# jinggqu/NextGen-UIA

Hardware: AMD Instinct MI355X
Metric: images/sec fwd+bwd BiomedCLIP+Mona bs=256 (higher is better)
Workload: dtype bf16

## Files before the change

include/uia_hip.h:

```cpp
#ifndef UIA_HIP_H
#define UIA_HIP_H
#include <stddef.h>
#include <stdint.h>

#ifdef __cplusplus
extern "C" {
#endif

enum { UIA_F32 = 0, UIA_BF16 = 1 };
enum { UIA_ACT_NONE = 0, UIA_ACT_GELU = 1, UIA_ACT_QUICKGELU = 2, UIA_ACT_RELU = 3 };
enum { UIA_MASK_NONE = 0, UIA_MASK_CAUSAL = 1, UIA_MASK_KEYPAD = 2 };
enum { UIA_MONA_BASELINE = 0, UIA_MONA_NOISE_AWARE = 1, UIA_MONA_FREQ_ENHANCED = 2, UIA_MONA_HYBRID = 3 };

const char* uia_last_error(void);
int uia_version(void);

typedef struct uia_gemm_desc {
    const void* A; int64_t lda;
    const void* W; int64_t ldw;
    int32_t M, N, K;
    float alpha;
    const float* bias;
    int32_t act;
    int32_t dact;
    const void* aux_in; int64_t ldaux_in;
    void* aux_out; int64_t ldaux_out;
    const float* resid; int64_t ldr;
    int32_t resid_mod, resid_row_off;
    const void* residT; int64_t ldrT;
    int32_t out_group;
    void* outT; int64_t ldo;
    float* out32; int64_t ldo32;
    int32_t w_kblocked;
    const void* resid_ln_stats;
    const float* resid_ln_w;
    const float* resid_ln_b;
    int64_t* rowsum_out;
    const int64_t* lnfold_sums;
    const float* lnfold_colsum;
    int32_t lnfold_dim; float lnfold_eps;
    int32_t resid_ln_dim; float resid_ln_eps;
    int64_t a_kb_rows;
    int64_t outT_kb_rows;
    int32_t* ln_flag;
    float ln_flag_limit;
    int32_t drop_where;
    float drop_p;
    uint64_t drop_seed;
    void* a_drop_out;
    float* splitk_ws;
    const void* A2;
    int64_t lda2;
    int32_t K2;
    int32_t a2_group_cols;
    int64_t a2_group_stride;
    const int8_t* resid_lo8;
    int64_t ld_resid_lo;
    int64_t residT_kb_rows;
    int8_t* out_lo8;
    int64_t ld_out_lo;
    int64_t resid_lo_kb_rows;
    int64_t out_lo_kb_rows;
} uia_gemm_desc;
int uia_gemm(void* stream, int dtype, const uia_gemm_desc* d, int tile_cfg );

int uia_wgrad(void* stream, int dtype, int M, int I, int J, const void* A, int64_t lda, const void* B, int64_t ldb,
              float alpha, float* dW, float* dbias_A);
int uia_wgrad_ex(void* stream, int dtype, int M, int I, int J, const void* A, int64_t lda, const void* B, int64_t ldb,
                 float alpha, float* dW, int64_t ldw, int i_valid, int j_valid, float* dbias_A);
int uia_wgrad_drop(void* stream, int dtype, int M, int I, int J, const void* A, int64_t lda, const void* B, int64_t ldb,
                   float alpha, float* dW, int64_t ldw, int i_valid, int j_valid, float drop_p, uint64_t seed, int64_t drop_ld, int drop_col0);
typedef struct uia_wgrad_group_desc {
    int32_t n, M, I, J;
    const void* A[4];
    const void* B[4];
    float* dW[4];
    float* dbias_A[4];
    int64_t lda, ldb, ldw;
    int32_t i_valid, j_valid;
    float alpha, drop_p;
    uint64_t drop_seed[4];
    int64_t drop_ld;
    int32_t drop_col0, reserved;
} uia_wgrad_group_desc;
int uia_wgrad_group(void* stream, int dtype, const uia_wgrad_group_desc* d);

typedef struct uia_attn_desc {
    const void *q, *k, *v; int64_t ld_qkv;
    void* out; int64_t ldo;
    float* lse;
    const int32_t* keylen;
    int32_t B, H, L, dh;
    int32_t mask_kind;
// ... 286 lines not shown
```

nextgen-uia_amd/csrc/gemm.hip:

```cpp
#include "gemm_epilogue.h"

int uia_gemm_quad_launch(hipStream_t stream, const UiaGemmParams& p, bool specialise, int xflags);
int uia_gemm_quadv_launch(hipStream_t stream, const UiaGemmParams& p, bool specialise, int xflags, int depth);

namespace {

template <typename T, int BM, int BN, int WAVES_M, int WAVES_N>
__global__ __launch_bounds__(64 * WAVES_M * WAVES_N) void gemm_tn_kernel(const UiaGemmParams p) {
    extern __shared__ __attribute__((aligned(16))) char smem[];
    constexpr int NW = WAVES_M * WAVES_N;
    constexpr int WTM = BM / WAVES_M, WTN = BN / WAVES_N;
    constexpr int MT = WTM / 16, NT = WTN / 16;
    constexpr int A_BYTES = BM * 128, W_BYTES = BN * 128, BUF_BYTES = A_BYTES + W_BYTES;
    constexpr int A_PER_WAVE = (BM / 8) / NW, W_PER_WAVE = (BN / 8) / NW;
    static_assert((BM / 8) % NW == 0 && (BN / 8) % NW == 0, "staging must divide over the waves");
    static_assert(WTM % 16 == 0 && WTN % 16 == 0 && (NT % 2) == 0, "wave tile shape");
    constexpr int ESZ = (int)sizeof(T);

    const int tid = threadIdx.x, lane = tid & 63;
    const int wave = __builtin_amdgcn_readfirstlane(tid >> 6);
    const int wm = wave / WAVES_N, wn = wave % WAVES_N;

    const int tiles_n = (p.N + BN - 1) / BN;
    const int nwg = gridDim.x;
// ... 726 lines not shown
            if (t + PD < ntl) stage(t + PD);
            load_frags(buf);
            if (grp == 1 && t + 1 < ntl) retire(t + 1);
            UIA_SLOT_END();
            compute();
            if (grp == 0 && t + 1 < ntl) retire(t + 1);
            UIA_SLOT_END();
        }
        if (grp == 0) {
            UIA_SLOT_END();
        }
        const int cm0 = m0, cn0 = n0;
        const int next = tile + nslots;
        const bool more = next < t_hi;
        if (more) {
            point_at(next);
            for (int t = 0; t < PD && t < ntl; ++t) stage(t);
        }
        constexpr bool LNROW = EPI == EPI_GENERIC || (EPI & EPI_LNFOLD) != 0;
        gemm_epilogue_lds<T, MT, NT, WTM, WTN, EPI, true>(p, acc, smem + (NBUF - 1) * BUF_BYTES, wave, lane, cm0, cn0, wm, wn,
                                                          LNROW ? (float*)(smem + NBUF * BUF_BYTES + wave * (WTM * 8)) : nullptr);
        if (!more) break;
        tile = next;
    }
#undef UIA_SLOT_END
}

template <typename T, int EPI>
int launch_persist_epi(hipStream_t stream, const UiaGemmParams& p) {
    constexpr int LDS = 4 * 512 * 64 + ((EPI == EPI_GENERIC || (EPI & EPI_LNFOLD) != 0) ? 4 * 256 * 8 : 0);
    auto kern = gemm_tn_persist_kernel<T, EPI>;
    static UiaDevOnce attr_once;
    UIA_ENSURE_LDS_ATTR(attr_once, kern, LDS);
    const int tiles = ((p.M + 255) / 256) * ((p.N + 255) / 256);
    const int ncu = uia_num_cus();
    hipLaunchKernelGGL(kern, dim3(tiles < ncu ? tiles : ncu), dim3(512), LDS, stream, p);
    UIA_CHECK_LAUNCH();
    return 0;
}


template <typename T, int BM, int BN, int WAVES_M, int WAVES_N, int BKB, int NBUF, int LOOP = 0>
int launch_ring(hipStream_t stream, const UiaGemmParams& p, bool specialise, int xflags, int sk_info = 0) {
    if constexpr (BM == 128 && BN == 256 && NBUF == 4 && LOOP == 0) {
        if (sk_info != 0) return launch_ring_epi<T, BM, BN, WAVES_M, WAVES_N, BKB, NBUF, EPI_GENERIC, LOOP, true>(stream, p, xflags, sk_info);
    }
    if constexpr (BN == 256 && NBUF == 4 && LOOP == 0 && BKB == 64 && sizeof(T) == 2) {
        if (p.K2 > 0) {
            switch (epi_mask_of(p)) {
                case EPI_BIAS | EPI_OUTT: return launch_ring_epi<T, BM, BN, WAVES_M, WAVES_N, BKB, NBUF, (EPI_BIAS | EPI_OUTT), LOOP, false, true>(stream, p, xflags);
                case EPI_OUTT: return launch_ring_epi<T, BM, BN, WAVES_M, WAVES_N, BKB, NBUF, (EPI_OUTT), LOOP, false, true>(stream, p, xflags);
                case EPI_BIAS | EPI_RESID | EPI_OUT32: return launch_ring_epi<T, BM, BN, WAVES_M, WAVES_N, BKB, NBUF, (EPI_BIAS | EPI_RESID | EPI_OUT32), LOOP, false, true>(stream, p, xflags);
                default: return launch_ring_epi<T, BM, BN, WAVES_M, WAVES_N, BKB, NBUF, EPI_GENERIC, LOOP, false, true>(stream, p, xflags);
            }
        }
    }
    if (specialise) {
        switch (epi_mask_of(p)) {
#define UIA_EPI_CASE(MASK) case (MASK): return launch_ring_epi<T, BM, BN, WAVES_M, WAVES_N, BKB, NBUF, (MASK), LOOP>(stream, p, xflags)
            UIA_EPI_CASE(EPI_BIAS | EPI_RESID | EPI_OUT32);
            UIA_EPI_CASE(EPI_BIAS | EPI_RESIDT | EPI_OUT32);
            UIA_EPI_CASE(EPI_BIAS | EPI_RESID | EPI_RESID_LN | EPI_OUT32);
            UIA_EPI_CASE(EPI_OUTT);
            UIA_EPI_CASE(EPI_BIAS | EPI_OUTT);
            UIA_EPI_CASE(EPI_BIAS | EPI_GELU | EPI_OUTT);
            UIA_EPI_CASE(EPI_DGELU | EPI_OUTT);
            UIA_EPI_CASE(EPI_BIAS | EPI_GELU | EPI_AUX_OUT | EPI_OUTT);
            UIA_EPI_CASE(EPI_QUICK | EPI_BIAS | EPI_GELU | EPI_OUTT);
            UIA_EPI_CASE(EPI_QUICK | EPI_DGELU | EPI_OUTT);
            UIA_EPI_CASE(EPI_QUICK | EPI_BIAS | EPI_GELU | EPI_AUX_OUT | EPI_OUTT);
            UIA_EPI_CASE(EPI_BIAS | EPI_RESID | EPI_OUT32 | EPI_OUTT | EPI_ROWSUM);
            UIA_EPI_CASE(EPI_BIAS | EPI_RESID | EPI_RESID_LN | EPI_OUT32 | EPI_OUTT | EPI_ROWSUM);
            UIA_EPI_CASE(EPI_BIAS | EPI_RESID_LO | EPI_RESID_LN | EPI_OUTT | EPI_OUT_LO | EPI_ROWSUM);
            UIA_EPI_CASE(EPI_BIAS | EPI_RESID | EPI_OUTT | EPI_OUT_LO | EPI_ROWSUM);
            UIA_EPI_CASE(EPI_BIAS | EPI_RESID_LO | EPI_OUT32);
            UIA_EPI_CASE(EPI_BIAS | EPI_RESID | EPI_RESID_LN | EPI_OUTT | EPI_OUT_LO | EPI_ROWSUM);
            UIA_EPI_CASE(EPI_BIAS | EPI_RESID_LO | EPI_RESID_LN | EPI_OUT32);
            UIA_EPI_CASE(EPI_BIAS | EPI_RESID_LO | EPI_OUT32 | EPI_OUTT | EPI_ROWSUM);
            UIA_EPI_CASE(EPI_BIAS | EPI_OUTT | EPI_LNFOLD);
            UIA_EPI_CASE(EPI_BIAS | EPI_GELU | EPI_OUTT | EPI_LNFOLD);
            UIA_EPI_CASE(EPI_BIAS | EPI_GELU | EPI_AUX_OUT | EPI_OUTT | EPI_LNFOLD);
            UIA_EPI_CASE(EPI_QUICK | EPI_BIAS | EPI_GELU | EPI_OUTT | EPI_LNFOLD);
            UIA_EPI_CASE(EPI_QUICK | EPI_BIAS | EPI_GELU | EPI_AUX_OUT | EPI_OUTT | EPI_LNFOLD);
#undef UIA_EPI_CASE
            default: break;
        }
    }
    return launch_ring_epi<T, BM, BN, WAVES_M, WAVES_N, BKB, NBUF, EPI_GENERIC, LOOP>(stream, p, xflags);
}

template <typename T>
int launch_persist(hipStream_t stream, const UiaGemmParams& p) {
    switch (epi_mask_of(p)) {
#define UIA_EPI_CASE(MASK) case (MASK): return launch_persist_epi<T, (MASK)>(stream, p)
        UIA_EPI_CASE(EPI_BIAS | EPI_RESID | EPI_OUT32);
        UIA_EPI_CASE(EPI_BIAS | EPI_RESIDT | EPI_OUT32);
        UIA_EPI_CASE(EPI_OUTT);
        UIA_EPI_CASE(EPI_BIAS | EPI_OUTT);
        UIA_EPI_CASE(EPI_BIAS | EPI_GELU | EPI_OUTT);
        UIA_EPI_CASE(EPI_DGELU | EPI_OUTT);
        UIA_EPI_CASE(EPI_BIAS | EPI_GELU | EPI_AUX_OUT | EPI_OUTT);
        UIA_EPI_CASE(EPI_BIAS | EPI_OUTT | EPI_LNFOLD);
        UIA_EPI_CASE(EPI_BIAS | EPI_GELU | EPI_OUTT | EPI_LNFOLD);
        UIA_EPI_CASE(EPI_BIAS | EPI_GELU | EPI_AUX_OUT | EPI_OUTT | EPI_LNFOLD);
#undef UIA_EPI_CASE
        default: break;
    }
    return launch_persist_epi<T, EPI_GENERIC>(stream, p);
}

template <int CH, int NWV = 8>
__global__ __launch_bounds__(64 * NWV) void gemm_skinny64_kernel(const UiaGemmParams p) {
    extern __shared__ __attribute__((aligned(16))) char smem[];
    const int K = p.K, KS = K >> 5;
    const int ldw_b = 2 * K + 16;
    const int tid = threadIdx.x, lane = tid & 63, li = lane & 15, g = lane >> 4;
    const int wave = __builtin_amdgcn_readfirstlane(tid >> 6);
    {
        const int cpr = K >> 3;
        for (int c = tid; c < 64 * cpr; c += 64 * NWV) {
            const int r = c / cpr, cc = c - r * cpr;
            *(uint4*)(smem + r * ldw_b + cc * 16) = *(const uint4*)((const char*)p.W + ((size_t)r * p.ldw) * 2 + cc * 16);
        }
    }
    __syncthreads();
    float bias[4][4];
#pragma unroll
    for (int nt = 0; nt < 4; ++nt)
#pragma unroll
        for (int r = 0; r < 4; ++r) bias[nt][r] = p.bias ? p.bias[16 * nt + 4 * g + r] : 0.f;
    const char* wfrag = smem + li * ldw_b + g * 16;
    const bool drop_a = p.drop_where == 1;
    const uint32_t drop_th = dropout_thresh16(p.drop_p);
    const float drop_inv = 1.0f / (1.0f - p.drop_p);
    const int ntiles = (p.M + 15) >> 4;
    for (int tile = wave * gridDim.x + blockIdx.x; tile < ntiles; tile += gridDim.x * NWV) {
        const int m = 16 * tile + li;
        const int mc = m < p.M ? m : p.M - 1;
        const char* arow = (const char*)p.A + ((size_t)mc * p.lda) * 2 + g * 16;
        f32x4 acc[4] = {f32x4{0.f, 0.f, 0.f, 0.f}, f32x4{0.f, 0.f, 0.f, 0.f}, f32x4{0.f, 0.f, 0.f, 0.f}, f32x4{0.f, 0.f, 0.f, 0.f}};
        for (int ks0 = 0; ks0 < KS; ks0 += CH) {
            uint4 a[CH];
#pragma unroll
            for (int i = 0; i < CH; ++i) a[i] = ks0 + i < KS ? *(const uint4*)(arow + (ks0 + i) * 64) : uint4{0u, 0u, 0u, 0u};
            if (drop_a) {
#pragma unroll
                for (int i = 0; i < CH; ++i) {
                    if (ks0 + i < KS) {
                        const uint32_t keep = dropout_keep8(p.drop_seed, (uint32_t)(((size_t)mc * (size_t)K + (size_t)((ks0 + i) * 32 + g * 8)) >> 3), drop_th);
                        bf16x8 v = __builtin_bit_cast(bf16x8, a[i]);
#pragma unroll
                        for (int e = 0; e < 8; ++e) v[e] = (bf16_t)((keep >> e) & 1u ? (float)v[e] * drop_inv : 0.f);
                        a[i] = __builtin_bit_cast(uint4, v);
                        if (p.a_drop_out && m < p.M) *(uint4*)((char*)p.a_drop_out + ((size_t)m * p.lda) * 2 + g * 16 + (ks0 + i) * 64) = a[i];
                    }
                }
            }
#pragma unroll
            for (int i = 0; i < CH; ++i) {
                if (ks0 + i < KS) {
#pragma unroll
                    for (int nt = 0; nt < 4; ++nt) {
                        const uint4 wf = *(const uint4*)(wfrag + nt * 16 * ldw_b + (ks0 + i) * 64);
                        acc[nt] = __builtin_amdgcn_mfma_f32_16x16x32_bf16(__builtin_bit_cast(bf16x8, wf), __builtin_bit_cast(bf16x8, a[i]), acc[nt], 0, 0, 0);
                    }
                }
// ... 220 lines not shown
        return -1;
    }
    if (p.w_kblocked && !ring) {
        uia_set_error("uia_gemm: a K-blocked W needs a ring tile config (8, 9, 10, 13), not %d", cfg);
        return -1;
    }
    if (ring) {
        int gm = gm_req == 255 ? 0 : gm_req;
        if (gm_req == 0) gm = p.N >= 1536 ? 8 : 0;
        xflags = (xflags & ~255) | gm;
    }
    switch (cfg) {
        case 1: return launch_cfg<T, 256, 256, 2, 4>(stream, p);
        case 2: return launch_cfg<T, 256, 128, 4, 2>(stream, p);
        case 3: return launch_cfg<T, 128, 128, 2, 2>(stream, p);
        case 4: return launch_cfg<T, 256, 64, 4, 1>(stream, p);
        case 5: return launch_cfg<T, 128, 64, 2, 1>(stream, p);
        case 21: return launch_cfg<T, 32, 64, 2, 2>(stream, p);
        case 23:
            if (!wide64_ok(p, (int)sizeof(T))) { uia_set_error("uia_gemm: tile cfg 23 is the bf16 K = 64 stream kernel (alpha, bias, accumulator dropout, one residual of the output's type)"); return -1; }
            return launch_wide64(stream, p);
        case 6: return launch_pp<T, 256, 256, 2, 4>(stream, p);
        case 7: return launch_pp<T, 256, 128, 4, 2>(stream, p);
        case 8: return launch_ring<T, 256, 256, 2, 4, 64, 4>(stream, p, true, xflags);
        case 9: return launch_ring<T, 256, 128, 4, 2, 128, 3>(stream, p, false, xflags);
        case 10: return launch_ring<T, 256, 256, 2, 4, 64, 4>(stream, p, false, xflags);
        case 12: return launch_persist<T>(stream, p);
        case 16:
            if (!skinny64_ok(p, (int)sizeof(T))) { uia_set_error("uia_gemm: tile cfg 16 is the bf16 N = 64 stream kernel (bias + T output only)"); return -1; }
            return launch_skinny64(stream, p);
#ifdef UIA_GEMM_EXP
        case 15: return launch_ring<T, 256, 256, 2, 4, 64, 4, 1>(stream, p, true, xflags);
#endif
#ifdef UIA_GEMM_EXP
        case 19: return launch_ring<T, 256, 256, 2, 4, 64, 4, 3>(stream, p, true, xflags);
        case 20: return launch_ring<T, 256, 256, 2, 4, 64, 4, 4>(stream, p, true, xflags);
#endif
#if defined(UIA_GEMM_EXP) || defined(UIA_GEMM_CFG1718)
        case 17: return launch_ring<T, 256, 128, 2, 2, 64, 3>(stream, p, true, xflags);
        case 18: return launch_ring<T, 128, 256, 1, 4, 64, 3>(stream, p, true, xflags);
#endif
        case 24: return launch_ring<T, 256, 256, 2, 4, 64, 5>(stream, p, true, xflags);
        case 25:
        case 26:
            if (sizeof(T) != 2) { uia_set_error("uia_gemm: tile cfg %d is bf16 only", cfg); return -1; }
            return uia_gemm_quad_launch(stream, p, cfg == 25, (xflags & 255) | (((cfg_in >> 16) & 7) << 8));
        case 27:
        case 28:
        case 29:
            if (sizeof(T) != 2) { uia_set_error("uia_gemm: tile cfg %d is bf16 only", cfg); return -1; }
            return uia_gemm_quadv_launch(stream, p, true, xflags & 255, cfg == 27 ? 2 : cfg == 28 ? 3 : 9);
        case 14: return launch_ring<T, 128, 256, 2, 4, 64, 3>(stream, p, true, xflags);
        case 13: return launch_ring<T, 128, 256, 2, 4, 64, 4>(stream, p, true, xflags, sk_info);
        default: uia_set_error("uia_gemm: unknown tile config %d", cfg); return -1;
    }
}

}

int uia_gemm_launch(hipStream_t stream, int dtype, const UiaGemmParams& p, int cfg) {
    const int esz = dtype == UIA_BF16 ? 2 : 4;
    const int bk = 128 / esz;
    UIA_CHECK_ARG(dtype == UIA_BF16 || dtype == UIA_F32, "uia_gemm: bad dtype %d", dtype);
    UIA_CHECK_ARG(p.M > 0 && p.N > 0 && p.K > 0, "uia_gemm: empty problem M=%d N=%d K=%d", p.M, p.N, p.K);
    UIA_CHECK_ARG(p.K % bk == 0, "uia_gemm: K=%d must be a multiple of %d for this dtype", p.K, bk);
    UIA_CHECK_ARG(p.N % 8 == 0, "uia_gemm: N=%d must be a multiple of 8", p.N);
    UIA_CHECK_ARG(p.A && p.W, "uia_gemm: null operand");
    UIA_CHECK_ARG((p.a_kb_rows || p.lda >= p.K - (p.K2 > 0 ? p.K2 : 0)) && p.ldw >= p.K, "uia_gemm: leading dimension smaller than K");
    UIA_CHECK_ARG((p.a_kb_rows || (p.lda * esz) % 16 == 0) && (p.ldw * esz) % 16 == 0, "uia_gemm: rows must be 16-byte aligned");
    UIA_CHECK_ARG(((uintptr_t)p.A % 16) == 0 && ((uintptr_t)p.W % 16) == 0, "uia_gemm: operands must be 16-byte aligned");
    UIA_CHECK_ARG(p.outT || p.out32, "uia_gemm: no output");
    UIA_CHECK_ARG(!p.outT || ((p.outT_kb_rows || p.ldo % 8 == 0) && (uintptr_t)p.outT % 16 == 0), "uia_gemm: outT alignment");
    UIA_CHECK_ARG(!p.out32 || (p.ldo32 % 4 == 0 && (uintptr_t)p.out32 % 16 == 0), "uia_gemm: out32 alignment");
    UIA_CHECK_ARG(!p.resid || (p.ldr % 4 == 0 && (uintptr_t)p.resid % 16 == 0), "uia_gemm: resid alignment");
    UIA_CHECK_ARG(!p.residT || ((p.residT_kb_rows || p.ldrT % 8 == 0) && (uintptr_t)p.residT % 16 == 0), "uia_gemm: residT alignment");
    UIA_CHECK_ARG(!p.resid_lo8 || (dtype == UIA_BF16 && p.residT && !p.resid && (p.resid_lo_kb_rows ? (p.resid_lo_kb_rows >= p.M && p.N % 64 == 0) : (p.ld_resid_lo >= p.N && p.ld_resid_lo % 8 == 0)) && (uintptr_t)p.resid_lo8 % 8 == 0 &&
                                  p.resid_mod == 0 && p.out_group == 0),
                  "uia_gemm: resid_lo8 needs bf16, residT as the hi plane, no fp32 resid, 8-byte aligned rows of at least N bytes and no row remapping");
    UIA_CHECK_ARG(p.residT_kb_rows == 0 || (p.resid_lo8 && p.residT_kb_rows >= p.M && (p.N * esz) % 64 == 0), "uia_gemm: residT_kb_rows needs resid_lo8, at least M rows and N*2 a multiple of 64");
    UIA_CHECK_ARG(!p.out_lo8 || (dtype == UIA_BF16 && p.outT && (p.out_lo_kb_rows ? (p.out_lo_kb_rows >= p.M && p.N % 64 == 0) : (p.ld_out_lo >= p.N && p.ld_out_lo % 8 == 0)) && (uintptr_t)p.out_lo8 % 8 == 0 && p.out_group == 0),
                  "uia_gemm: out_lo8 needs bf16, outT as the hi plane, 8-byte aligned rows of at least N bytes and no row remapping");
    UIA_CHECK_ARG(!p.bias || (uintptr_t)p.bias % 16 == 0, "uia_gemm: bias alignment");
    UIA_CHECK_ARG(!p.dact || p.aux_in, "uia_gemm: dact needs aux_in");
    UIA_CHECK_ARG(!p.aux_in || (p.ldaux_in % 8 == 0 && (uintptr_t)p.aux_in % 16 == 0), "uia_gemm: aux_in alignment");
    UIA_CHECK_ARG(!p.aux_out || (p.ldaux_out % 8 == 0 && (uintptr_t)p.aux_out % 16 == 0), "uia_gemm: aux_out alignment");
    UIA_CHECK_ARG(p.resid_mod == 0 || p.resid, "uia_gemm: resid_mod without resid");
    UIA_CHECK_ARG(!p.resid_ln_stats || ((p.resid || p.resid_lo8) && p.resid_ln_w && p.resid_ln_b), "uia_gemm: resid_ln_stats needs resid (or residT + resid_lo8), resid_ln_w and resid_ln_b");
    UIA_CHECK_ARG(!p.resid_ln_stats || ((uintptr_t)p.resid_ln_stats % 8 == 0 && (uintptr_t)p.resid_ln_w % 16 == 0 && (uintptr_t)p.resid_ln_b % 16 == 0),
                  "uia_gemm: resid_ln alignment");
    UIA_CHECK_ARG(p.a_kb_rows == 0 || p.a_kb_rows >= p.M, "uia_gemm: a_kb_rows=%lld < M=%d", (long long)p.a_kb_rows, p.M);
    UIA_CHECK_ARG(p.outT_kb_rows == 0 || (p.outT && p.outT_kb_rows >= p.M && (p.N * esz) % 64 == 0 && p.out_group == 0),
                  "uia_gemm: outT_kb_rows needs outT, at least M rows, N*sizeof(T) a multiple of 64 and no row remapping");
    UIA_CHECK_ARG(!p.resid_ln_stats || p.resid_ln_dim >= 0, "uia_gemm: resid_ln_dim=%d", p.resid_ln_dim);
    UIA_CHECK_ARG(!p.rowsum_out || ((uintptr_t)p.rowsum_out % 16 == 0 && p.out_group == 0), "uia_gemm: rowsum_out must be 16-byte aligned and takes no row remapping");
    UIA_CHECK_ARG(!(p.resid_ln_stats && p.resid_ln_dim > 0) || (uintptr_t)p.resid_ln_stats % 16 == 0, "uia_gemm: row sums behind resid_ln_stats must be 16-byte aligned");
    UIA_CHECK_ARG(!p.ln_flag || (uintptr_t)p.ln_flag % 4 == 0, "uia_gemm: ln_flag must be a 4-byte aligned device word");
    UIA_CHECK_ARG(p.drop_where >= 0 && p.drop_where <= 2, "uia_gemm: drop_where=%d (0 none, 1 A operand, 2 accumulator)", p.drop_where);
    UIA_CHECK_ARG(p.drop_where == 0 || (p.drop_p >= 0.f && p.drop_p < 1.f), "uia_gemm: drop_p=%f outside [0, 1)", (double)p.drop_p);
    UIA_CHECK_ARG(p.drop_where != 1 || (dtype == UIA_BF16 && (size_t)p.M * (size_t)p.K / 8 <= 0xFFFFFFFFull && (uintptr_t)p.a_drop_out % 16 == 0 && !p.a_kb_rows),
                  "uia_gemm: dropout on the A operand needs bf16, row-major A, M*K <= 2^35 and a 16-byte aligned a_drop_out");
    UIA_CHECK_ARG(p.drop_where != 2 || (size_t)p.M * (size_t)p.N / 8 <= 0xFFFFFFFFull, "uia_gemm: dropout on the accumulator needs M*N <= 2^35");
    UIA_CHECK_ARG(p.drop_where == 1 || !p.a_drop_out, "uia_gemm: a_drop_out without drop_where = 1");
    UIA_CHECK_ARG(p.K2 >= 0 && (p.K2 == 0 || (dtype == UIA_BF16 && p.A2 && p.K2 % 32 == 0 && p.K2 < p.K && p.lda2 >= p.K2 && (p.lda2 * 2) % 16 == 0 && (uintptr_t)p.A2 % 16 == 0 &&
                                             p.a2_group_cols >= 0 && p.a2_group_cols % 256 == 0 && !p.a_kb_rows && p.lda >= p.K - p.K2)),
                  "uia_gemm: the K extension needs bf16, a row-major A of K - K2 columns, a 16-byte aligned row-major A2 with K2 (a multiple of 32, < K) columns and "
                  "column groups that are multiples of 256; got K=%d K2=%d lda2=%lld group=%d", p.K, p.K2, (long long)p.lda2, p.a2_group_cols);
    UIA_CHECK_ARG(!p.lnfold_sums || (p.lnfold_colsum && p.lnfold_dim > 0 && p.alpha == 1.0f && (uintptr_t)p.lnfold_sums % 16 == 0 && (uintptr_t)p.lnfold_colsum % 16 == 0),
                  "uia_gemm: lnfold_sums needs lnfold_colsum (16-byte aligned), lnfold_dim > 0 and alpha == 1");
    UIA_CHECK_ARG(!p.outT || p.outT_kb_rows || p.ldo >= p.N, "uia_gemm: ldo=%lld < N=%d", (long long)p.ldo, p.N);
    UIA_CHECK_ARG(!p.out32 || p.ldo32 >= p.N, "uia_gemm: ldo32=%lld < N=%d", (long long)p.ldo32, p.N);
    UIA_CHECK_ARG(!p.aux_out || p.ldaux_out >= p.N, "uia_gemm: ldaux_out=%lld < N=%d", (long long)p.ldaux_out, p.N);
    UIA_CHECK_ARG(!p.aux_in || p.ldaux_in >= p.N, "uia_gemm: ldaux_in=%lld < N=%d", (long long)p.ldaux_in, p.N);
    UIA_CHECK_ARG(!p.resid || p.ldr >= p.N, "uia_gemm: ldr=%lld < N=%d", (long long)p.ldr, p.N);
    UIA_CHECK_ARG(!p.residT || p.residT_kb_rows || p.ldrT >= p.N, "uia_gemm: ldrT=%lld < N=%d", (long long)p.ldrT, p.N);
    if (dtype == UIA_BF16) return launch_typed<bf16_t>(stream, p, cfg);
    return launch_typed<float>(stream, p, cfg);
}
```

nextgen-uia_amd/csrc/gemm_epilogue.h:

```cpp
#pragma once
#include "uia_common.h"
#include "uia_kernels.h"

#ifdef UIA_GEMM_STAMPS
static __device__ unsigned long long* uia_stamp_buf = nullptr;
static __device__ int uia_epi_diag = 0;
#define UIA_EPI_STORES ((uia_epi_diag & 3) == 0)
#define UIA_EPI_LOADS ((uia_epi_diag & 3) < 2)
#ifndef UIA_KDIAG
#define UIA_KDIAG 0
#endif
#define UIA_DIAG_NO_FRAGS ((UIA_KDIAG & 4) != 0)
#define UIA_DIAG_NO_DMA ((UIA_KDIAG & 8) != 0)
#define UIA_DIAG_NO_MFMA ((UIA_KDIAG & 16) != 0)
#else
#define UIA_EPI_STORES true
#define UIA_EPI_LOADS true
#define UIA_DIAG_NO_FRAGS false
#define UIA_DIAG_NO_DMA false
#define UIA_DIAG_NO_MFMA false
#endif

namespace {

template <typename T> struct MfmaTile;

template <> struct MfmaTile<bf16_t> {
    static __device__ __forceinline__ f32x4 mma(const uint4& w, const uint4& a, f32x4 c) {
        return __builtin_amdgcn_mfma_f32_16x16x32_bf16(__builtin_bit_cast(bf16x8, w),
                                                       __builtin_bit_cast(bf16x8, a), c, 0, 0, 0);
    }
};
template <> struct MfmaTile<float> {
    static __device__ __forceinline__ f32x4 mma(const uint4& w, const uint4& a, f32x4 c) {
        c = __builtin_amdgcn_mfma_f32_16x16x4f32(__builtin_bit_cast(float, w.x), __builtin_bit_cast(float, a.x), c, 0, 0, 0);
        c = __builtin_amdgcn_mfma_f32_16x16x4f32(__builtin_bit_cast(float, w.y), __builtin_bit_cast(float, a.y), c, 0, 0, 0);
        c = __builtin_amdgcn_mfma_f32_16x16x4f32(__builtin_bit_cast(float, w.z), __builtin_bit_cast(float, a.z), c, 0, 0, 0);
        c = __builtin_amdgcn_mfma_f32_16x16x4f32(__builtin_bit_cast(float, w.w), __builtin_bit_cast(float, a.w), c, 0, 0, 0);
        return c;
    }
};

template <bool FAST>
__device__ __forceinline__ float apply_act(float x, int act) {
    switch (act) {
        case UIA_ACT_GELU: return gelu_erf_t<FAST>(x);
        case UIA_ACT_QUICKGELU: return quick_gelu(x);
        case UIA_ACT_RELU: return fmaxf(x, 0.0f);
        default: return x;
    }
}
template <bool FAST>
__device__ __forceinline__ void apply_act8(float (&v)[8], int act) {
    if (FAST && act == UIA_ACT_GELU) {
#pragma unroll
        for (int e = 0; e < 8; e += 2) {
            const f32x2 x = {v[e], v[e + 1]}, y = gelu_poly2(x);
            v[e] = y[0];
            v[e + 1] = y[1];
        }
    } else {
#pragma unroll
        for (int e = 0; e < 8; ++e) v[e] = apply_act<FAST>(v[e], act);
    }
}
template <bool FAST>
__device__ __forceinline__ float apply_dact(float pre, int act);
template <bool FAST>
__device__ __forceinline__ void apply_dact8(float (&v)[8], const float (&a)[8], int act) {
    if (FAST && act == UIA_ACT_GELU) {
#pragma unroll
        for (int e = 0; e < 8; e += 2) {
            const f32x2 x = {a[e], a[e + 1]}, d = dgelu_poly2(x);
            v[e] *= d[0];
            v[e + 1] *= d[1];
        }
    } else {
#pragma unroll
        for (int e = 0; e < 8; ++e) v[e] *= apply_dact<FAST>(a[e], act);
    }
}
template <bool FAST>
__device__ __forceinline__ float apply_dact(float pre, int act) {
    switch (act) {
        case UIA_ACT_GELU: return dgelu_erf_t<FAST>(pre);
        case UIA_ACT_QUICKGELU: return dquick_gelu(pre);
        case UIA_ACT_RELU: return pre > 0.0f ? 1.0f : 0.0f;
        default: return 1.0f;
    }
}

__device__ __forceinline__ void glds16(const char* gsrc, char* lds_wave_base) {
    __builtin_amdgcn_global_load_lds((const __attribute__((address_space(1))) void*)gsrc,
                                     (__attribute__((address_space(3))) void*)lds_wave_base, 16, 0, 0);
}

__device__ __forceinline__ void glds16_asm(const char* gsrc, char* lds_wave_base) {
    const unsigned dst = (unsigned)(uintptr_t)(__attribute__((address_space(3))) char*)lds_wave_base;
    const unsigned dst_u = __builtin_amdgcn_readfirstlane(dst);
    unsigned keep;
    asm volatile("s_mov_b32 %0, m0\n\ts_mov_b32 m0, %2\n\ts_nop 0\n\tglobal_load_lds_dwordx4 %1, off\n\ts_mov_b32 m0, %0"
                 : "=&s"(keep)
                 : "v"(gsrc), "s"(dst_u)
                 : "memory");
}

typedef long long2 __attribute__((ext_vector_type(2)));
constexpr float ROWSUM_SCALE = 1073741824.0f, ROWSUM_INV = 1.0f / 1073741824.0f;
constexpr float ROWSUM_PART_MAX = 5.0e8f;
__device__ __forceinline__ void rowsum_add(void* dst, size_t row, float s1, float s2, int* flag) {
    if (!(fabsf(s1) < ROWSUM_PART_MAX) || !(s2 < ROWSUM_PART_MAX)) {
        if (flag) atomicOr(flag, 2);
        s1 = fminf(fmaxf(s1, -ROWSUM_PART_MAX), ROWSUM_PART_MAX);
        s2 = fminf(fmaxf(s2, 0.0f), ROWSUM_PART_MAX);
    }
    unsigned long long* q = (unsigned long long*)dst + 2 * row;
    atomicAdd(q, (unsigned long long)llrintf(s1 * ROWSUM_SCALE));
    atomicAdd(q + 1, (unsigned long long)llrintf(s2 * ROWSUM_SCALE));
}
__device__ __forceinline__ float2 rowsum_load(const void* src, size_t row) {
    const long2 v = *(const long2*)((const long long*)src + 2 * row);
    return float2{(float)v[0] * ROWSUM_INV, (float)v[1] * ROWSUM_INV};
}
struct LnRow { float mean, rstd, nmr; };
__device__ __forceinline__ LnRow ln_row_from_sums(float2 ss, int dim, float eps) {
    const float inv = 1.0f / (float)dim;
    const float mean = ss.x * inv;
    const float var = fmaxf(fmaf(-mean, mean, ss.y * inv), 0.0f);
    const float rstd = rsqrtf(var + eps);
    return LnRow{mean, rstd, -mean * rstd};
}
__device__ __forceinline__ void ln_fold_guard(const UiaGemmParams& p, const LnRow& ln) {
    if (p.ln_flag && fabsf(ln.nmr) > (p.ln_flag_limit > 0.f ? p.ln_flag_limit : 8.0f)) atomicOr(p.ln_flag, 1);
}

template <int LPR>
__device__ __forceinline__ float row_lanes_sum(float v) {
    if constexpr (LPR == 8) {
        v += __builtin_bit_cast(float, __builtin_amdgcn_update_dpp(0, __builtin_bit_cast(int, v), 0xB1, 0xF, 0xF, true));
        v += __builtin_bit_cast(float, __builtin_amdgcn_update_dpp(0, __builtin_bit_cast(int, v), 0x4E, 0xF, 0xF, true));
        v += __builtin_bit_cast(float, __builtin_amdgcn_update_dpp(0, __builtin_bit_cast(int, v), 0x141, 0xF, 0xF, true));
    } else {
#pragma unroll
        for (int o = 1; o < LPR; o <<= 1) v += __shfl_xor(v, o);
    }
    return v;
}

template <typename T, int MT, int NT, int WTM, int WTN>
__device__ __forceinline__ void gemm_epilogue(const UiaGemmParams& p, f32x4 (&acc)[MT][NT], int m0, int n0, int wm, int wn, int li, int g) {
    const int nb = n0 + wn * WTN + g * (4 * NT);
    T* outT = (T*)p.outT;
    const T* aux_in = (const T*)p.aux_in;
    T* aux_out = (T*)p.aux_out;
    const T* residT = (const T*)p.residT;
#pragma unroll
    for (int i = 0; i < MT; ++i) {
        const int m = m0 + wm * WTM + 16 * i + li;
        if (m >= p.M) continue;
        const size_t orow = p.out_group > 0 ? (size_t)(m + m / p.out_group + 1) : (size_t)m;
        const size_t rrow = p.resid_mod > 0 ? (size_t)(m % p.resid_mod + p.resid_row_off) : orow;
#pragma unroll
        for (int jj = 0; jj < NT; jj += 2) {
            const int n = nb + 4 * jj;
            if (n >= p.N) continue;
            float v[8];
#pragma unroll
            for (int e = 0; e < 4; ++e) { v[e] = acc[i][jj][e] * p.alpha; v[4 + e] = acc[i][jj + 1][e] * p.alpha; }
            if (p.lnfold_sums) {
                const float2 ss = rowsum_load(p.lnfold_sums, (size_t)m);
                const LnRow ln = ln_row_from_sums(ss, p.lnfold_dim, p.lnfold_eps);
                if (jj == 0 && nb == 0) ln_fold_guard(p, ln);
                float cs[8];
                load8(p.lnfold_colsum + n, cs);
#pragma unroll
                for (int e = 0; e < 8; ++e) v[e] = fmaf(v[e], ln.rstd, ln.nmr * cs[e]);
            }
            if (p.bias) {
                float b[8];
                load8(p.bias + n, b);
#pragma unroll
                for (int e = 0; e < 8; ++e) v[e] += b[e];
            }
            if (aux_out) store8(aux_out + orow * p.ldaux_out + n, v);
            if (p.act) {
                apply_act8<sizeof(T) == 2>(v, p.act);
            }
            if (p.dact) {
                float a[8];
                load8(aux_in + orow * p.ldaux_in + n, a);
                apply_dact8<sizeof(T) == 2>(v, a, p.dact);
            }
            if (p.drop_where == 2) {
                const uint32_t keep = dropout_keep8(p.drop_seed, (uint32_t)(((size_t)m * (size_t)p.N + (size_t)n) >> 3), dropout_thresh16(p.drop_p));
                const float inv_keep = 1.0f / (1.0f - p.drop_p);
#pragma unroll
                for (int e = 0; e < 8; ++e) v[e] = (keep >> e) & 1u ? v[e] * inv_keep : 0.f;
            }
            if (p.resid) {
                float r[8];
                load8(p.resid + rrow * p.ldr + n, r);
                if (p.resid_ln_stats) {
                    float2 ms;
                    if (p.resid_ln_dim > 0) { const LnRow ln = ln_row_from_sums(rowsum_load(p.resid_ln_stats, rrow), p.resid_ln_dim, p.resid_ln_eps); ms = float2{ln.mean, ln.rstd}; }
                    else ms = *(const float2*)((const float*)p.resid_ln_stats + 2 * rrow);
                    float lw[8], lb[8];
                    load8(p.resid_ln_w + n, lw);
                    load8(p.resid_ln_b + n, lb);
#pragma unroll
                    for (int e = 0; e < 8; ++e) r[e] = fmaf((r[e] - ms.x) * ms.y, lw[e], lb[e]);
                }
#pragma unroll
                for (int e = 0; e < 8; ++e) v[e] += r[e];
            }
            if (residT) {
                float r[8];
                load8(residT + orow * p.ldrT + n, r);
#pragma unroll
                for (int e = 0; e < 8; ++e) v[e] += r[e];
            }
            if (p.out32) store8(p.out32 + orow * p.ldo32 + n, v);
            if (outT) store8(outT + orow * p.ldo + n, v);
            if (p.rowsum_out) {
                float s1 = 0.f, s2 = 0.f;
#pragma unroll
                for (int e = 0; e < 8; ++e) { s1 += v[e]; s2 = fmaf(v[e], v[e], s2); }
                rowsum_add(p.rowsum_out, orow, s1, s2, p.ln_flag);
            }
        }
    }
}


template <int MT, int WTN> struct EpiPatch {
    static constexpr int LDW = WTN + 4;
    static constexpr int GPP = MT < 4 ? MT : (MT == 4 ? 2 : 4);
    static constexpr int ROWS = GPP * 16;
    static constexpr int BYTES_PER_WAVE = ROWS * LDW * 4;
};

enum : int { EPI_BIAS = 1, EPI_AUX_OUT = 2, EPI_GELU = 4, EPI_DGELU = 8, EPI_RESID = 16, EPI_RESIDT = 32, EPI_OUT32 = 64, EPI_OUTT = 128,
             EPI_RESID_LN = 256,
             EPI_ROWSUM = 512,
             EPI_LNFOLD = 1024,
             EPI_QUICK = 2048,
             EPI_RESID_LO = 4096,
             EPI_OUT_LO = 8192,
             EPI_GENERIC = -1 };

template <typename T, int MT, int NT, int WTM, int WTN, int EPI = EPI_GENERIC, bool PATCH16 = false, int WCOLS = 4>
__device__ __forceinline__ void gemm_epilogue_lds(const UiaGemmParams& p, f32x4 (&acc)[MT][NT], char* smem, int wave, int lane, int m0, int n0,
                                                  int wm, int wn, float* lnrow_lds = nullptr, const float2* lnpre = nullptr) {
    constexpr bool GEN = EPI == EPI_GENERIC;
    const bool f_bias = GEN ? p.bias != nullptr : (EPI & EPI_BIAS) != 0;
    const bool f_aux_out = GEN ? p.aux_out != nullptr : (EPI & EPI_AUX_OUT) != 0;
    const bool f_resid = GEN ? p.resid != nullptr : (EPI & EPI_RESID) != 0;
    const bool f_rlo = GEN ? p.resid_lo8 != nullptr : (EPI & EPI_RESID_LO) != 0;
    const bool f_olo = GEN ? p.out_lo8 != nullptr : (EPI & EPI_OUT_LO) != 0;
    const bool f_residT = GEN ? (p.residT != nullptr && p.resid_lo8 == nullptr) : ((EPI & EPI_RESIDT) != 0 && (EPI & EPI_RESID_LO) == 0);
    const bool f_rln = GEN ? ((p.resid != nullptr || p.resid_lo8 != nullptr) && p.resid_ln_stats != nullptr) : (EPI & EPI_RESID_LN) != 0;
    const bool f_out32 = GEN ? p.out32 != nullptr : (EPI & EPI_OUT32) != 0;
    const bool f_outT = GEN ? p.outT != nullptr : (EPI & EPI_OUTT) != 0;
    const bool f_rowsum = GEN ? p.rowsum_out != nullptr : (EPI & EPI_ROWSUM) != 0;
    const bool f_lnfold = GEN ? p.lnfold_sums != nullptr : (EPI & EPI_LNFOLD) != 0;
    const int act = GEN ? p.act : ((EPI & EPI_GELU) ? ((EPI & EPI_QUICK) ? UIA_ACT_QUICKGELU : UIA_ACT_GELU) : UIA_ACT_NONE);
    const int dact = GEN ? p.dact : ((EPI & EPI_DGELU) ? ((EPI & EPI_QUICK) ? UIA_ACT_QUICKGELU : UIA_ACT_GELU) : UIA_ACT_NONE);
    using EP = EpiPatch<MT, WTN>;
    constexpr int LDW = EP::LDW, GPP = EP::GPP, ROWS = EP::ROWS;
    constexpr int LPR = WTN / 8;
    constexpr int RPP = 64 / LPR;
    static_assert(MT % GPP == 0, "row groups must split evenly into phases");
    const int li = lane & 15, g = lane >> 4;
    const int rr = lane / LPR, rc = (lane % LPR) * 8;
    const int n = n0 + wn * WTN + rc;
    T* outT = (T*)p.outT;
    const T* aux_in = (const T*)p.aux_in;
    T* aux_out = (T*)p.aux_out;
    const T* residT = (const T*)p.residT;
    float bias[8];
#pragma unroll
    for (int e = 0; e < 8; ++e) bias[e] = 0.f;
    if (f_bias && n < p.N) load8(p.bias + n, bias);
    const bool col_ok = n < p.N;
    float lnw[8], lnb[8];
#pragma unroll
    for (int e = 0; e < 8; ++e) { lnw[e] = 1.f; lnb[e] = 0.f; }
    if (f_rln && col_ok) { load8(p.resid_ln_w + n, lnw); load8(p.resid_ln_b + n, lnb); }
    float csum[8];
#pragma unroll
    for (int e = 0; e < 8; ++e) csum[e] = 0.f;
    if (f_lnfold && col_ok) load8(p.lnfold_colsum + n, csum);
    const int mrow0 = m0 + wm * WTM;
    const bool rln_staged = f_rln && !f_lnfold && lnrow_lds != nullptr && lnpre != nullptr && !(GEN && (p.resid_mod > 0 || p.out_group > 0));
    if (rln_staged) {
#pragma unroll
        for (int i = 0; i < (WTM + 63) / 64; ++i) {
            const int r = lane + 64 * i;
            if (r < WTM) {
                float2 ms = lnpre[i];
                if (p.resid_ln_dim > 0) { const LnRow ln = ln_row_from_sums(ms, p.resid_ln_dim, p.resid_ln_eps); ms = float2{ln.mean, ln.rstd}; }
                *(float2*)(lnrow_lds + 2 * r) = ms;
            }
        }
    }
    if (f_lnfold && lnrow_lds) {
#pragma unroll
        for (int i = 0; i < (WTM + 63) / 64; ++i) {
            const int r = lane + 64 * i, m = mrow0 + r;
            if (r < WTM) {
                const float2 ss = lnpre ? lnpre[i] : (m < p.M ? rowsum_load(p.lnfold_sums, (size_t)m) : float2{0.f, 1.f});
                const LnRow ln = ln_row_from_sums(ss, p.lnfold_dim, p.lnfold_eps);
                if (wn == 0 && n0 == 0 && m < p.M) ln_fold_guard(p, ln);
                *(float2*)(lnrow_lds + 2 * r) = float2{ln.rstd, ln.nmr};
            }
        }
    }

    auto apply = [&](const f32x4& lo, const f32x4& hi, int m, const bf16x8* pre_aux = nullptr, const f32x4* pre_res = nullptr,
                     const bf16x8* pre_rt = nullptr, float* os1 = nullptr, float* os2 = nullptr, const uint2* pre_lo = nullptr) {
        const bool ok = m < p.M && col_ok;
        if (!f_rowsum && !ok) return;
        float v[8] = {lo[0], lo[1], lo[2], lo[3], hi[0], hi[1], hi[2], hi[3]};
        const size_t orow = GEN && p.out_group > 0 ? (size_t)(m + m / p.out_group + 1) : (size_t)m;
        const size_t rrow = GEN && p.resid_mod > 0 ? (size_t)(m % p.resid_mod + p.resid_row_off) : orow;
        if (ok) {
        if (f_lnfold) {
            float2 st;
            if (lnrow_lds) st = *(const float2*)(lnrow_lds + 2 * (m - mrow0));
            else { const LnRow ln = ln_row_from_sums(rowsum_load(p.lnfold_sums, (size_t)m), p.lnfold_dim, p.lnfold_eps); st = float2{ln.rstd, ln.nmr}; if (n == 0) ln_fold_guard(p, ln); }
            const f32x2 rs = {st.x, st.x}, nm = {st.y, st.y};
#pragma unroll
            for (int e = 0; e < 8; e += 2) {
                const f32x2 c2 = {csum[e], csum[e + 1]}, b2 = {bias[e], bias[e + 1]}, a2 = {v[e], v[e + 1]};
                const f32x2 r2 = __builtin_elementwise_fma(a2, rs, __builtin_elementwise_fma(nm, c2, b2));
                v[e] = r2[0];
                v[e + 1] = r2[1];
            }
        } else if (GEN) {
#pragma unroll
            for (int e = 0; e < 8; ++e) v[e] = fmaf(v[e], p.alpha, bias[e]);
        } else if (f_bias) {
#pragma unroll
            for (int e = 0; e < 8; ++e) v[e] += bias[e];
        }
        if (f_aux_out && UIA_EPI_STORES) store8(aux_out + orow * p.ldaux_out + n, v);
        if (act) apply_act8<sizeof(T) == 2>(v, act);
        if (dact && UIA_EPI_LOADS) {
            float a[8];
            if (pre_aux) {
#pragma unroll
                for (int e = 0; e < 8; ++e) a[e] = (float)(*pre_aux)[e];
            } else {
                load8(aux_in + orow * p.ldaux_in + n, a);
            }
            apply_dact8<sizeof(T) == 2>(v, a, dact);
        }
        if (GEN && p.drop_where == 2) {
            const uint32_t keep = dropout_keep8(p.drop_seed, (uint32_t)(((size_t)m * (size_t)p.N + (size_t)n) >> 3), dropout_thresh16(p.drop_p));
            const float inv_keep = 1.0f / (1.0f - p.drop_p);
#pragma unroll
            for (int e = 0; e < 8; ++e) v[e] = (keep >> e) & 1u ? v[e] * inv_keep : 0.f;
        }
        if ((f_resid || f_rlo) && UIA_EPI_LOADS) {
            float r[8];
            if (f_rlo) {
                typedef __attribute__((ext_vector_type(8))) unsigned short u16x8;
                u16x8 hv;
                uint2 lv;
                if (pre_rt) { hv = __builtin_bit_cast(u16x8, *pre_rt); lv = *pre_lo; }
                else {
                    constexpr int G = 64 / (int)sizeof(T);
                    const T* hp = p.residT_kb_rows ? residT + ((size_t)(n / G) * (size_t)p.residT_kb_rows + rrow) * G + (n % G) : residT + rrow * p.ldrT + n;
                    hv = *(const u16x8*)hp;
                    lv = *(const uint2*)(p.resid_lo_kb_rows ? p.resid_lo8 + (((size_t)(n >> 6) * (size_t)p.resid_lo_kb_rows + rrow) << 6) + (n & 63) : p.resid_lo8 + rrow * p.ld_resid_lo + n);
                }
#pragma unroll
                for (int e = 0; e < 8; ++e) {
                    const int lb = __builtin_amdgcn_sbfe((int)(e < 4 ? lv.x : lv.y), 8 * (e & 3), 8);
                    r[e] = __builtin_bit_cast(float, ((unsigned)hv[e] << 16) + ((unsigned)lb << 8));
                }
            } else if (pre_res) {
#pragma unroll
                for (int e = 0; e < 4; ++e) { r[e] = pre_res[0][e]; r[4 + e] = pre_res[1][e]; }
            } else {
                load8(p.resid + rrow * p.ldr + n, r);
            }
            if (f_rln) {
                float2 ms;
                if (rln_staged) ms = *(const float2*)(lnrow_lds + 2 * (m - mrow0));
                else if (p.resid_ln_dim > 0) { const LnRow ln = ln_row_from_sums(rowsum_load(p.resid_ln_stats, rrow), p.resid_ln_dim, p.resid_ln_eps); ms = float2{ln.mean, ln.rstd}; }
                else ms = *(const float2*)((const float*)p.resid_ln_stats + 2 * rrow);
#pragma unroll
                for (int e = 0; e < 8; ++e) r[e] = fmaf((r[e] - ms.x) * ms.y, lnw[e], lnb[e]);
            }
#pragma unroll
            for (int e = 0; e < 8; ++e) v[e] += r[e];
        }
        if (f_residT && UIA_EPI_LOADS) {
            float r[8];
            if (pre_rt) {
#pragma unroll
                for (int e = 0; e < 8; ++e) r[e] = (float)(*pre_rt)[e];
            } else {
                load8(residT + orow * p.ldrT + n, r);
            }
#pragma unroll
            for (int e = 0; e < 8; ++e) v[e] += r[e];
        }
        if (f_out32 && UIA_EPI_STORES) store8(p.out32 + orow * p.ldo32 + n, v);
        if (f_olo && UIA_EPI_STORES) {
            unsigned w[8];
#pragma unroll
            for (int e = 0; e < 8; ++e) {
                const unsigned vb = __builtin_bit_cast(unsigned, v[e]);
                const unsigned hb = (unsigned)__builtin_bit_cast(unsigned short, (bf16_t)v[e]);
                int d = (int)((vb + 0x80u) >> 8) - (int)(hb << 8);
                d = d < -127 ? -127 : (d > 127 ? 127 : d);
                w[e] = (unsigned)d & 0xFFu;
            }
            uint2 pk;
            pk.x = w[0] | (w[1] << 8) | (w[2] << 16) | (w[3] << 24);
            pk.y = w[4] | (w[5] << 8) | (w[6] << 16) | (w[7] << 24);
            *(uint2*)(p.out_lo_kb_rows ? p.out_lo8 + (((size_t)(n >> 6) * (size_t)p.out_lo_kb_rows + orow) << 6) + (n & 63) : p.out_lo8 + orow * p.ld_out_lo + n) = pk;
        }
        if (f_outT && UIA_EPI_STORES) {
            if (p.outT_kb_rows) {
                constexpr int G = 64 / (int)sizeof(T);
                store8(outT + ((size_t)(n / G) * (size_t)p.outT_kb_rows + orow) * G + (n % G), v);
            } else {
                store8(outT + orow * p.ldo + n, v);
// ... 68 lines not shown
                if (lcol_ok) { float t8[8]; load8(p.lnfold_colsum + nl, t8);
#pragma unroll
                    for (int e = 0; e < 8; ++e) c16[e] = t8[e]; }
                if (lcol_ok2) { float t8[8]; load8(p.lnfold_colsum + nl + 8, t8);
#pragma unroll
                    for (int e = 0; e < 8; ++e) c16[8 + e] = t8[e]; }
            }
            auto bounce = [&](int ph, int which) {
#pragma clang loop unroll(full)
                for (int gi = 0; gi < GPP; ++gi) {
                    const int i = ph * GPP + gi;
                    const int mloc = 16 * i + li;
                    float2 st = float2{1.f, 0.f};
                    if (f_lnfold) st = *(const float2*)(lnrow_lds + 2 * mloc);
                    const f32x2 rs2 = {st.x, st.x}, nm2 = {st.y, st.y};
                    bf16x8 outv[2];
#pragma unroll
                    for (int hf = 0; hf < 2; ++hf) {
                        float v[8] = {acc[i][2 * hf][0], acc[i][2 * hf][1], acc[i][2 * hf][2], acc[i][2 * hf][3],
                                      acc[i][2 * hf + 1][0], acc[i][2 * hf + 1][1], acc[i][2 * hf + 1][2], acc[i][2 * hf + 1][3]};
                        if (f_lnfold) {
#pragma unroll
                            for (int e = 0; e < 8; e += 2) {
                                const f32x2 c2 = {c16[8 * hf + e], c16[8 * hf + e + 1]}, bb2 = {b16[8 * hf + e], b16[8 * hf + e + 1]}, a2 = {v[e], v[e + 1]};
                                const f32x2 r2 = __builtin_elementwise_fma(a2, rs2, __builtin_elementwise_fma(nm2, c2, bb2));
                                v[e] = r2[0];
                                v[e + 1] = r2[1];
                            }
                        } else if (f_bias) {
#pragma unroll
                            for (int e = 0; e < 8; ++e) v[e] += b16[8 * hf + e];
                        }
                        if (which == 0 && act) apply_act8<true>(v, act);
                        const f32x4 lo = {v[0], v[1], v[2], v[3]}, hi = {v[4], v[5], v[6], v[7]};
                        bf16x8 r = {(bf16_t)lo[0], (bf16_t)lo[1], (bf16_t)lo[2], (bf16_t)lo[3], (bf16_t)hi[0], (bf16_t)hi[1], (bf16_t)hi[2], (bf16_t)hi[3]};
                        outv[hf] = r;
                    }
#ifdef UIA_EPI_DIRECT
                    {
                        T* dbase = which == 0 ? outT : aux_out;
                        const int m = m0 + wm * WTM + mloc;
                        if (m < p.M && UIA_EPI_STORES) {
                            T* d = (which == 0 && p.outT_kb_rows) ? dbase + ((size_t)(nl / 32) * (size_t)p.outT_kb_rows + (size_t)m) * 32 + (nl % 32)
                                                                  : dbase + (size_t)m * (which == 0 ? p.ldo : p.ldaux_out) + nl;
                            if (lcol_ok) *(bf16x8*)d = outv[0];
                            if (lcol_ok2) *(bf16x8*)(d + 8) = outv[1];
                        }
                    }
                    continue;
#endif
                    *(bf16x8*)(stb + (gi * 16 + li) * LDB + g * 32) = outv[0];
                    *(bf16x8*)(stb + (gi * 16 + li) * LDB + g * 32 + 16) = outv[1];
                }
#ifdef UIA_EPI_DIRECT
                return;
#endif
                asm volatile("s_waitcnt lgkmcnt(0)" ::: "memory");
                __builtin_amdgcn_wave_barrier();
                T* dstbase = which == 0 ? outT : aux_out;
                const int mbase = m0 + wm * WTM + ph * ROWS + rr;
#pragma unroll
                for (int q = 0; q < NPASS; ++q) {
                    const int row = q * RPP + rr;
                    const int m = mbase + q * RPP;
                    const bf16x8 val = *(const bf16x8*)(stb + row * LDB + rc * 2);
                    if (m < p.M && col_ok && UIA_EPI_STORES) {
                        if (which == 0 && p.outT_kb_rows) {
                            constexpr int G = 32;
                            *(bf16x8*)(dstbase + ((size_t)(n / G) * (size_t)p.outT_kb_rows + (size_t)m) * G + (n % G)) = val;
                        } else {
                            *(bf16x8*)(dstbase + (size_t)m * (which == 0 ? p.ldo : p.ldaux_out) + n) = val;
                        }
                    }
                }
                __builtin_amdgcn_wave_barrier();
            };
#pragma clang loop unroll(full)
            for (int ph = 0; ph < NPH; ++ph) {
                if (f_aux_out) bounce(ph, 1);
                bounce(ph, 0);
            }
        } else
        if constexpr (PIPE && NPASS % 2 == 0) {
            constexpr bool H_AUX = (EPI & EPI_DGELU) != 0, H_RES = (EPI & EPI_RESID) != 0, H_LO = (EPI & EPI_RESID_LO) != 0, H_RT = (EPI & EPI_RESIDT) != 0 || H_LO,
                           H_SUM = (EPI & EPI_ROWSUM) != 0;
            constexpr int CH = NPASS / 2, NCH = 2 * NPH;
            bf16x8 pa[2][H_AUX ? CH : 1];
            f32x4 pr[2][H_RES ? 2 * CH : 1];
            bf16x8 prt[2][H_RT ? CH : 1];
            uint2 plo[2][H_LO ? CH : 1];
            float rs1[H_SUM ? NCH * CH : 1], rs2[H_SUM ? NCH * CH : 1];
            const int mrow = m0 + wm * WTM + rr;
            const int nc = col_ok ? n : 0;
            auto issue = [&](int c, int set) {
                if (!UIA_EPI_LOADS) return;
#pragma unroll
                for (int q = 0; q < CH; ++q) {
                    const int m = mrow + (c * CH + q) * RPP;
                    const size_t mc = (size_t)(m < p.M ? m : p.M - 1);
                    if constexpr (H_AUX) pa[set][q] = *(const bf16x8*)((const bf16_t*)p.aux_in + mc * p.ldaux_in + nc);
                    if constexpr (H_RES) { const float* src = p.resid + mc * p.ldr + nc; pr[set][2 * q] = *(const f32x4*)src; pr[set][2 * q + 1] = *(const f32x4*)(src + 4); }
                    if constexpr (H_LO) {
                        const bf16_t* hp = p.residT_kb_rows ? (const bf16_t*)p.residT + ((size_t)(nc / 32) * (size_t)p.residT_kb_rows + mc) * 32 + (nc % 32)
                                                            : (const bf16_t*)p.residT + mc * p.ldrT + nc;
                        prt[set][q] = *(const bf16x8*)hp;
                        plo[set][q] = *(const uint2*)(p.resid_lo_kb_rows ? p.resid_lo8 + (((size_t)(nc >> 6) * (size_t)p.resid_lo_kb_rows + mc) << 6) + (nc & 63) : p.resid_lo8 + mc * p.ld_resid_lo + nc);
                    } else if constexpr (H_RT) prt[set][q] = *(const bf16x8*)((const bf16_t*)p.residT + mc * p.ldrT + nc);
                }
            };
            issue(0, 0);
            issue(1, 1);
#pragma clang loop unroll(full)
            for (int c = 0; c < NCH; ++c) {
                const int ph = c / 2, set = c & 1;
                if ((c & 1) == 0) {
#pragma clang loop unroll(full)
                    for (int gi = 0; gi < GPP; ++gi)
#pragma clang loop unroll(full)
                        for (int j = 0; j < NT; ++j) *(f32x4*)(stg + (gi * 16 + li) * LDW + g * (4 * NT) + 4 * j) = acc[ph * GPP + gi][j];
                    asm volatile("s_waitcnt lgkmcnt(0)" ::: "memory");
                    __builtin_amdgcn_wave_barrier();
                }
#pragma unroll
                for (int q = 0; q < CH; ++q) {
                    const int row = ((c & 1) * CH + q) * RPP + rr;
                    const f32x4 lo = *(const f32x4*)(stg + row * LDW + rc), hi = *(const f32x4*)(stg + row * LDW + rc + 4);
                    apply(lo, hi, mrow + (c * CH + q) * RPP, H_AUX ? &pa[set][q] : nullptr, H_RES ? &pr[set][2 * q] : nullptr, H_RT ? &prt[set][q] : nullptr,
                          H_SUM ? &rs1[c * CH + q] : nullptr, H_SUM ? &rs2[c * CH + q] : nullptr, H_LO ? &plo[set][q] : nullptr);
                }
                if (c + 2 < NCH) issue(c + 2, set);
                if ((c & 1) == 1) __builtin_amdgcn_wave_barrier();
            }
            if constexpr (H_SUM) {
                static_assert(WTN == 64, "64-column wave tiles");
                constexpr int RW = 2 * WTM;
                auto to_fixed = [&](float v, bool sq) -> long long {
                    if (!(fabsf(v) < ROWSUM_PART_MAX)) {
                        if (p.ln_flag) atomicOr(p.ln_flag, 2);
                        v = fminf(fmaxf(v, sq ? 0.0f : -ROWSUM_PART_MAX), ROWSUM_PART_MAX);
                    }
                    return llrintf(v * ROWSUM_SCALE);
                };
                long long* ex = (long long*)smem;
                __syncthreads();
                if ((lane % LPR) == 0) {
#pragma unroll
                    for (int k = 0; k < NCH * CH; ++k) {
                        long long* d = ex + wave * RW + 2 * (k * RPP + rr);
                        d[0] = to_fixed(rs1[k], false);
                        d[1] = to_fixed(rs2[k], true);
                    }
                }
                __syncthreads();
                const int nwaves = (int)(blockDim.x >> 6), wm_n = nwaves / WCOLS;
                for (int idx = wave * 64 + lane; idx < wm_n * RW; idx += nwaves * 64) {
                    const int wmr = idx / RW, off = idx - wmr * RW;
                    const long long* src = ex + (wmr * WCOLS) * RW + off;
                    long long v = src[0];
#pragma unroll
                    for (int c = 1; c < WCOLS; ++c) v += src[c * RW];
                    const int m = m0 + wmr * WTM + (off >> 1);
                    if (m < p.M) atomicAdd((unsigned long long*)p.rowsum_out + 2 * (size_t)m + (off & 1), (unsigned long long)v);
                }
            }
        } else {
#pragma clang loop unroll(full)
        for (int ph = 0; ph < MT / GPP; ++ph) {
#pragma clang loop unroll(full)
            for (int gi = 0; gi < GPP; ++gi)
#pragma clang loop unroll(full)
                for (int j = 0; j < NT; ++j) *(f32x4*)(stg + (gi * 16 + li) * LDW + g * (4 * NT) + 4 * j) = acc[ph * GPP + gi][j];
            asm volatile("s_waitcnt lgkmcnt(0)" ::: "memory");
            __builtin_amdgcn_wave_barrier();
            const int mbase = m0 + wm * WTM + ph * ROWS + rr;
#pragma clang loop unroll_count(2)
            for (int q = 0; q < ROWS / RPP; ++q) {
                const int row = q * RPP + rr;
                const f32x4 lo = *(const f32x4*)(stg + row * LDW + rc), hi = *(const f32x4*)(stg + row * LDW + rc + 4);
                apply(lo, hi, mbase + q * RPP);
            }
            __builtin_amdgcn_wave_barrier();
        }
        }
    }
}

inline int epi_mask_of(const UiaGemmParams& p) {
    if (p.alpha != 1.0f || p.out_group > 0 || p.resid_mod > 0 || p.drop_where == 2) return EPI_GENERIC;
    const bool quick = p.act == UIA_ACT_QUICKGELU || p.dact == UIA_ACT_QUICKGELU;
    if ((p.act && p.act != UIA_ACT_GELU && p.act != UIA_ACT_QUICKGELU) || (p.dact && p.dact != UIA_ACT_GELU && p.dact != UIA_ACT_QUICKGELU) ||
        (p.act && p.dact && p.act != p.dact)) return EPI_GENERIC;
    return (quick ? EPI_QUICK : 0) | (p.bias ? EPI_BIAS : 0) | (p.aux_out ? EPI_AUX_OUT : 0) | (p.act ? EPI_GELU : 0) | (p.dact ? EPI_DGELU : 0) | (p.resid ? EPI_RESID : 0) |
           ((p.resid && p.resid_ln_stats) ? EPI_RESID_LN : 0) | (p.rowsum_out ? EPI_ROWSUM : 0) | (p.lnfold_sums ? EPI_LNFOLD : 0) |
           ((p.residT && !p.resid_lo8) ? EPI_RESIDT : 0) | (p.out32 ? EPI_OUT32 : 0) | (p.outT ? EPI_OUTT : 0) |
           (p.resid_lo8 ? EPI_RESID_LO : 0) | ((p.resid_lo8 && p.resid_ln_stats) ? EPI_RESID_LN : 0) | (p.out_lo8 ? EPI_OUT_LO : 0);
}

}
```

nextgen-uia_amd/csrc/uia_common.h:

```cpp
#pragma once
#include <hip/hip_runtime.h>
#include <stdint.h>

typedef __bf16 bf16_t;
typedef __attribute__((ext_vector_type(8))) __bf16 bf16x8;
typedef __attribute__((ext_vector_type(4))) __bf16 bf16x4;
typedef __attribute__((ext_vector_type(2))) __bf16 bf16x2;
typedef __attribute__((ext_vector_type(4))) float f32x4;

#define UIA_WAVE 64

void uia_set_error(const char* fmt, ...);
#define UIA_CHECK_ARG(cond, ...)                 \
    do {                                         \
        if (!(cond)) {                           \
            uia_set_error(__VA_ARGS__);          \
            return -1;                           \
        }                                        \
    } while (0)
#define UIA_CHECK_HIP(expr)                                                              \
    do {                                                                                 \
        hipError_t _e = (expr);                                                          \
        if (_e != hipSuccess) {                                                          \
            uia_set_error("%s failed: %s (%s:%d)", #expr, hipGetErrorString(_e),         \
                          __FILE__, __LINE__);                                           \
            return -2;                                                                   \
        }                                                                                \
    } while (0)
#define UIA_CHECK_LAUNCH() UIA_CHECK_HIP(hipGetLastError())

#include <atomic>
struct UiaDevOnce {
    std::atomic<unsigned long long> mask{0};
};
#define UIA_ENSURE_LDS_ATTR(once, kern, bytes)                                                                     \
    do {                                                                                                           \
        int _dev = 0;                                                                                              \
        UIA_CHECK_HIP(hipGetDevice(&_dev));                                                                        \
        const unsigned long long _bit = 1ull << (_dev & 63);                                                       \
        if (!((once).mask.load(std::memory_order_acquire) & _bit)) {                                               \
            UIA_CHECK_HIP(hipFuncSetAttribute((const void*)(kern), hipFuncAttributeMaxDynamicSharedMemorySize, (bytes))); \
            (once).mask.fetch_or(_bit, std::memory_order_release);                                                 \
        }                                                                                                          \
    } while (0)

#if defined(__HIPCC__)
__device__ __forceinline__ f32x4 three_byte_load4(const bf16_t* hi, const int8_t* lo) {
    typedef __attribute__((ext_vector_type(4))) unsigned short u16x4;
    const u16x4 h = *(const u16x4*)hi;
    const int l = *(const int*)lo;
    f32x4 r;
#pragma unroll
    for (int e = 0; e < 4; ++e) r[e] = __builtin_bit_cast(float, ((unsigned)h[e] << 16) + ((unsigned)__builtin_amdgcn_sbfe(l, 8 * e, 8) << 8));
    return r;
}
__device__ __forceinline__ void three_byte_store4(bf16_t* hi, int8_t* lo, f32x4 v) {
    unsigned w[4];
    unsigned short hs[4];
    const float f[4] = {v[0], v[1], v[2], v[3]};
#pragma unroll
    for (int e = 0; e < 4; ++e) {
        const unsigned vb = __builtin_bit_cast(unsigned, f[e]);
        hs[e] = __builtin_bit_cast(unsigned short, (bf16_t)f[e]);
        int d = (int)((vb + 0x80u) >> 8) - (int)((unsigned)hs[e] << 8);
        d = d < -127 ? -127 : (d > 127 ? 127 : d);
        w[e] = (unsigned)d & 0xFFu;
    }
    uint2 hp;
    hp.x = (unsigned)hs[0] | ((unsigned)hs[1] << 16);
    hp.y = (unsigned)hs[2] | ((unsigned)hs[3] << 16);
    *(uint2*)hi = hp;
    *(unsigned*)lo = w[0] | (w[1] << 8) | (w[2] << 16) | (w[3] << 24);
}

__device__ __forceinline__ f32x4 three_byte_decode4(uint2 hraw, unsigned lraw) {
    const unsigned h[4] = {hraw.x & 0xFFFFu, hraw.x >> 16, hraw.y & 0xFFFFu, hraw.y >> 16};
    f32x4 r;
#pragma unroll
    for (int e = 0; e < 4; ++e) r[e] = __builtin_bit_cast(float, (h[e] << 16) + ((unsigned)__builtin_amdgcn_sbfe((int)lraw, 8 * e, 8) << 8));
    return r;
}

#endif

inline int uia_num_cus() {
    static int n = 0;
    if (n == 0) {
        int dev = 0;
        hipDeviceProp_t prop;
        n = (hipGetDevice(&dev) == hipSuccess && hipGetDeviceProperties(&prop, dev) == hipSuccess && prop.multiProcessorCount > 0)
                ? prop.multiProcessorCount : 256;
    }
    return n;
}

__device__ __forceinline__ float to_f32(float x) { return x; }
__device__ __forceinline__ float to_f32(bf16_t x) { return (float)x; }

template <typename T> __device__ __forceinline__ T from_f32(float x);
template <> __device__ __forceinline__ float from_f32<float>(float x) { return x; }
template <> __device__ __forceinline__ bf16_t from_f32<bf16_t>(float x) { return (bf16_t)x; }

__device__ __forceinline__ f32x4 load4(const float* p) { return *(const f32x4*)p; }
__device__ __forceinline__ f32x4 load4(const bf16_t* p) {
    bf16x4 v = *(const bf16x4*)p;
    f32x4 r = {(float)v[0], (float)v[1], (float)v[2], (float)v[3]};
    return r;
}
__device__ __forceinline__ void store4(float* p, f32x4 v) { *(f32x4*)p = v; }
__device__ __forceinline__ void store4(bf16_t* p, f32x4 v) {
    bf16x4 r = {(bf16_t)v[0], (bf16_t)v[1], (bf16_t)v[2], (bf16_t)v[3]};
    *(bf16x4*)p = r;
}
__device__ __forceinline__ void load8(const float* p, float (&o)[8]) {
    f32x4 a = *(const f32x4*)p, b = *(const f32x4*)(p + 4);
    o[0] = a[0]; o[1] = a[1]; o[2] = a[2]; o[3] = a[3];
    o[4] = b[0]; o[5] = b[1]; o[6] = b[2]; o[7] = b[3];
}
__device__ __forceinline__ void load8(const bf16_t* p, float (&o)[8]) {
    bf16x8 v = *(const bf16x8*)p;
#pragma unroll
    for (int i = 0; i < 8; ++i) o[i] = (float)v[i];
}
__device__ __forceinline__ void store8(float* p, const float (&v)[8]) {
    f32x4 a = {v[0], v[1], v[2], v[3]}, b = {v[4], v[5], v[6], v[7]};
    *(f32x4*)p = a;
    *(f32x4*)(p + 4) = b;
}
__device__ __forceinline__ void store8(bf16_t* p, const float (&v)[8]) {
    bf16x8 r;
#pragma unroll
    for (int i = 0; i < 8; ++i) r[i] = (bf16_t)v[i];
    *(bf16x8*)p = r;
}

template <bool FAST>
__device__ __forceinline__ void gelu_parts(float x, float& Phi, float& E) {
    const float ax = fabsf(x) * 0.70710678118654752f;
    E = __expf(-ax * ax);
    float y;
    if (FAST) {
        const float t = __builtin_amdgcn_rcpf(fmaf(0.47047f, ax, 1.0f));
        y = fmaf(fmaf(0.7478556f, t, -0.0958798f), t, 0.3480242f) * t;
    } else {
        const float t = __builtin_amdgcn_rcpf(fmaf(0.3275911f, ax, 1.0f));
        y = fmaf(1.061405429f, t, -1.453152027f);
        y = fmaf(y, t, 1.421413741f);
        y = fmaf(y, t, -0.284496736f);
        y = fmaf(y, t, 0.254829592f) * t;
    }
    const float half_erfc = 0.5f * y * E;
    Phi = x >= 0.f ? 1.0f - half_erfc : half_erfc;
}
template <bool FAST = false> __device__ __forceinline__ float gelu_erf_t(float x) {
    float P, E;
    gelu_parts<FAST>(x, P, E);
    return x * P;
}
template <bool FAST = false> __device__ __forceinline__ float dgelu_erf_t(float x) {
    float P, E;
    gelu_parts<FAST>(x, P, E);
    return fmaf(x * 0.39894228040143268f, E, P);
}
__device__ __forceinline__ float gelu_erf(float x) { return gelu_erf_t<false>(x); }
__device__ __forceinline__ float dgelu_erf(float x) { return dgelu_erf_t<false>(x); }
// ... 104 lines not shown
```

nextgen-uia_amd/uia_hip/functional.py:

```python
import math
import os
import weakref

import time

import torch

from . import handoff, ops
from ._lib import UiaError
from .handoff import (ClsGrad, Resid3, _g3_partner_feeds, cls_grad_of, fwd3_of, grad3_decode, grad3_of, grad_resid3_enabled, hook_free, linear_chain,
                      publish_cls_grad, publish_fwd3, publish_grad3, publish_rows, publish_t_copy, set_cls_grad, set_grad_resid3, t_copy_of, take_rows, zero_sums,
                      cls_only, set_cls_forward, take_cls_forward)
from .handoff import clear as clear_t_copies

_STATE = {"dtype": torch.bfloat16, "seed": 0x5EED, "calls": 0, "fwd_resid3": os.environ.get("UIA_FWD_RESID3", "1") != "0"}


def set_compute_dtype(dt):
    assert dt in (torch.bfloat16, torch.float32)
    _STATE["dtype"] = dt


def compute_dtype():
    return _STATE["dtype"]


def set_deferred_text_ln(flag):
    _STATE["text_ln_deferred"] = bool(flag)


def set_block_resid3(flag):
    _STATE["block_resid3"] = bool(flag)


def set_fwd_resid3(flag):
    _STATE["fwd_resid3"] = bool(flag)


def set_text_resid3(flag):
    _STATE["text_resid3"] = bool(flag)


def set_ln_fold(flag):
    _STATE["ln_fold"] = bool(flag)


def set_deterministic(flag):
    _STATE["deterministic"] = bool(flag)
    ops.TAIL_SPLIT_K = not flag


def ln_fold_enabled(dt, rows=None):
    return dt != torch.float32 and _STATE.get("ln_fold", True) and (rows is None or rows > _STATE.get("ln_fold_min_rows", 2048))


class LnFoldRangeError(FloatingPointError):
    """A GEMM that left row sums for a folded LayerNorm saw a non-finite or out-of-range partial sum: the LayerNorm statistics of that
    row — and everything downstream of it — are wrong."""


_FOLD_POLL = {}
_FOLD_REPORTED = {}


POLL_LAG = max(1, int(os.environ.get("UIA_POLL_LAG", "2")))


def reset_ln_flag(device=None):
    dev = torch.device("cuda", torch.cuda.current_device()) if device is None else torch.device(device)
    key = dev.index if dev.index is not None else torch.cuda.current_device()
    _FOLD_POLL.pop(key, None)
    _FOLD_REPORTED.pop(key, None)
    if key in ops._LN_FLAG:
        ops._LN_FLAG[key].zero_()


def poll_ln_flag(device=None, sync=False):
    dev = torch.device("cuda", torch.cuda.current_device()) if device is None else torch.device(device)
    key = dev.index if dev.index is not None else torch.cuda.current_device()
    flag = ops._LN_FLAG.get(key)
    if flag is None:
        return 0
    seen = 0
    pending = _FOLD_POLL.setdefault(key, [])
    while pending and (sync or len(pending) >= POLL_LAG):
        prev = pending.pop(0)
        t0 = time.perf_counter()
        prev[1].synchronize()
        _STATE["gpu_wait_s"] = _STATE.get("gpu_wait_s", 0.0) + time.perf_counter() - t0
        seen |= int(prev[0][0])
    host = torch.empty(1, dtype=torch.int32, pin_memory=True)
    host.copy_(flag, non_blocking=True)
    ev = torch.cuda.Event()
    ev.record()
    if sync:
        ev.synchronize()
        seen |= int(host[0])
    else:
        pending.append((host, ev))
    seen &= ~_FOLD_REPORTED.get(key, 0) | 2
    _FOLD_REPORTED[key] = _FOLD_REPORTED.get(key, 0) | (seen & 1)
    if seen & 2:
        raise LnFoldRangeError("uia_hip: a LayerNorm row sum was non-finite or out of the fixed-point range (|Σ| or Σ² >= 5e8 in one column "
                               "block): the activations have diverged; the statistics of that row are not valid")
    if seen & 1 and _STATE.get("ln_fold", True):
        import warnings
        warnings.warn(f"uia_hip: LayerNorm fold switched off: a row with |mean| / std > {ops.LN_FLAG_LIMIT} would lose bf16 precision as a raw "
                      "GEMM operand; the LayerNorm kernels are used from the next forward on")
        set_ln_fold(False)
    return seen


def set_fp32_heads(flag):
    _STATE["fp32_heads"] = bool(flag)


def head_dtype():
    return torch.float32 if _STATE.get("fp32_heads", True) else compute_dtype()


def set_unpad_text(flag):
    _STATE["unpad_text"] = bool(flag)

# ... 433 lines not shown
    _STATE["wgrad_side_stream"] = bool(flag)


def join_side_streams():
    cur = torch.cuda.current_stream()
    for st in _WGRAD_SIDE.values():
        cur.wait_stream(st)


DIRECT_TRAIN = True


def _is_flat_grad(p):
    g = p.grad
    return (getattr(p, "_uia_flat_grad", False) and g is not None and g.dtype == torch.float32 and g.is_contiguous() and g.shape == p.shape
            and g.device == p.device)


def mona_apply(x_bnd, module_params, variant, hw, p_drop, training, keep_mask=None):
    names = tuple(k for k in MONA_PARAM_ORDER if k in module_params)
    pd = p_drop if (training or keep_mask is not None) else 0.0
    params = [module_params[k] for k in names]
    direct = torch.is_grad_enabled() and all(p.requires_grad and _is_flat_grad(p) for p in params)
    return MonaFn.apply(x_bnd, variant, tuple(hw), pd, keep_mask, names, direct, *params)


class BlockSpec:

    def __init__(self, heads, eps, act, ln1, qkv, proj, ln2, fc1, fc2, mask=None, publish_out=False):
        self.heads, self.eps, self.act, self.mask = heads, eps, act, mask
        self.publish_out = publish_out
        self.ln1, self.qkv, self.proj, self.ln2, self.fc1, self.fc2 = ln1, qkv, proj, ln2, fc1, fc2


ATTN_SINGLE_PASS_MAX = 272


class VitBlockFn(torch.autograd.Function):

    @staticmethod
    def forward(ctx, x, spec):
        B, N, D = x.shape
        M, dt = B * N, compute_dtype()
        if N > ATTN_SINGLE_PASS_MAX and (ctx.needs_input_grad[0] or spec.mask is not None):
            raise UiaError(f"vit_block: {N} tokens exceed the {ATTN_SINGLE_PASS_MAX} of the attention backward; sequences this long run forward-only "
                           "(frozen tower under torch.no_grad()), unmasked" if ctx.needs_input_grad[0] else
                           f"vit_block: {N} tokens with a mask: the long attention forward takes no mask")
        x3 = fwd3_of(x)
        like = x3.lo if x3 is not None else x
        if x3 is None:
            x = x.contiguous()
            x2d = x.view(M, D)
        train = ctx.needs_input_grad[0]
        fold = ln_fold_enabled(dt, M)
        if x3 is not None:
            assert fold and dt == torch.bfloat16, "a three-byte forward token reached a block that cannot take it"
            rows = (x3.hi, x3.sums)
        else:
            rows = take_rows(x, dt) if fold else None
        qkv = _empty((M, 3 * D), dt, like)
        if rows is not None:
            wq, cq, bq = WEIGHTS.get_lnfold(spec.qkv[0], spec.qkv[1], spec.ln1[0], spec.ln1[1], dt)
            xin_t, sums0 = rows
            if not ops.is_kb(xin_t):
                xin_t = xin_t.view(M, D)
            ops.gemm(xin_t, wq, bias=bq, out_t=qkv, lnfold=(sums0, cq, D, spec.eps))
            h1 = _act(M, D, dt, like, spec.fc1[0].shape[0]) if x3 is not None else xin_t
        else:
            h1 = _empty((M, D), dt, x)
            ops.layernorm_fwd(x2d, spec.ln1[0], spec.ln1[1], spec.eps, y_t=h1)
            ops.gemm(h1, WEIGHTS.get(spec.qkv[0], dt), bias=spec.qkv[1], out_t=qkv)
        if handoff.take_last_block_cls() and spec.mask is None and 1 < N <= ATTN_SINGLE_PASS_MAX and D == 64 * spec.heads and like.is_cuda:
            return VitBlockFn._forward_cls(ctx, x, x3, qkv, spec, (B, N, D), dt, train)
        if N > ATTN_SINGLE_PASS_MAX:
            a = _empty((M, D), dt, like)
            ops.attn_fwd_long(qkv[:, :D], qkv[:, D:2 * D], qkv[:, 2 * D:], a, B, spec.heads, N)
            lse = None
        else:
            a = _attn_act(M, D, dt, like, D) if D == 64 * spec.heads else _empty((M, D), dt, like)
            lse = torch.empty(B, spec.heads, N, device=like.device, dtype=torch.float32) if train else None
            ops.attn_fwd(qkv[:, :D], qkv[:, D:2 * D], qkv[:, 2 * D:], a, B, spec.heads, N, lse=lse, mask=spec.mask)
        F = spec.fc1[0].shape[0]
        f = _act(M, F, dt, like, D)
        pre = _empty((M, F), dt, like) if train else None
        r3 = fold and _STATE.get("block_resid3", False) and dt == torch.bfloat16 and M > 2048
        x1 = None if r3 else torch.empty(M, D, device=like.device, dtype=torch.float32)
        lo1 = torch.empty(M, D, device=like.device, dtype=torch.int8) if r3 else None
        if fold:
            sums1 = zero_sums(M, like.device)
            h1 = _as_act(h1, M, D, dt, F) if x3 is None else h1
            resx = dict(resid3=x3.resid3) if x3 is not None else dict(resid=x2d)
            ops.gemm(a, WEIGHTS.get(spec.proj[0], dt), bias=spec.proj[1], out32=x1, out_t=h1, out_lo=lo1, rowsum=sums1, **resx)
            w1, c1, b1 = WEIGHTS.get_lnfold(spec.fc1[0], spec.fc1[1], spec.ln2[0], spec.ln2[1], dt)
            ops.gemm(h1, w1, bias=b1, act=spec.act, aux_out=pre, out_t=f, lnfold=(sums1, c1, D, spec.eps))
        else:
            ops.gemm(a, WEIGHTS.get(spec.proj[0], dt), bias=spec.proj[1], resid=x2d, out32=x1)
            h1 = _as_act(h1, M, D, dt, 0)
            ops.layernorm_fwd(x1, spec.ln2[0], spec.ln2[1], spec.eps, y_t=h1)
            ops.gemm(h1, WEIGHTS.get(spec.fc1[0], dt), bias=spec.fc1[1], act=spec.act, aux_out=pre, out_t=f)
        x2 = torch.empty(B, N, D, device=like.device, dtype=torch.float32)
        res1 = dict(resid3=Resid3(h1, lo1)) if r3 else dict(resid=x1)
        if fold and spec.publish_out:
            sums2 = zero_sums(M, like.device)
            h2 = _act(M, D, dt, like, 3 * D) if r3 else _as_act(h1, M, D, dt, 3 * D)
            ops.gemm(f, WEIGHTS.get(spec.fc2[0], dt), bias=spec.fc2[1], out32=x2.view(M, D), out_t=h2, rowsum=sums2, **res1)
            publish_rows(x2, h2, sums2)
        else:
            ops.gemm(f, WEIGHTS.get(spec.fc2[0], dt), bias=spec.fc2[1], out32=x2.view(M, D), **res1)
        if train:
            saved, ctx.layout = handoff.save_layout(x3.resid3 if x3 is not None else x, qkv, a, lse, Resid3(h1, lo1) if r3 else x1, pre)
            ctx.save_for_backward(*saved)
            ctx.xshape = (B, N, D)
            ctx.spec = spec
            ctx.g3_out = dt == torch.bfloat16 and _g3_partner_feeds(x)
            ctx.cls_ok = spec.mask is None and N <= ATTN_SINGLE_PASS_MAX and D == 64 * spec.heads and not r3 and handoff.cls_grad_enabled()
        return x2

    @staticmethod
    def _forward_cls(ctx, x, x3, qkv, spec, shape, dt, train):
        B, N, D = shape
        like = qkv
        a = _empty((B, D), dt, like)
        lse = torch.empty(B, spec.heads, device=like.device, dtype=torch.float32) if train else None
        ops.attn_fwd_cls(qkv[:, :D], qkv[:, D:2 * D], qkv[:, 2 * D:], a, B, spec.heads, N, lse=lse)
        x_cls = torch.empty(B, D, device=like.device, dtype=torch.float32)
        if x3 is not None:
            ops.rows3_to_f32(x3.hi, x3.lo, N, x_cls)
        else:
            ops.copy_rows(x.view(B * N, D), N, x_cls)
        x1 = torch.empty(B, D, device=like.device, dtype=torch.float32)
        M = B * N
        wp = WEIGHTS.get(spec.proj[0], dt)
        ops.gemm(a, wp, bias=spec.proj[1], resid=x_cls, out32=x1, tile_cfg=_rows_tile_cfg(M, wp, like, dt, out32=True, resid=True))
        h2 = _empty((B, D), dt, like)
        ops.layernorm_fwd(x1, spec.ln2[0], spec.ln2[1], spec.eps, y_t=h2)
        F = spec.fc1[0].shape[0]
        f = _empty((B, F), dt, like)
        pre = _empty((B, F), dt, like) if train else None
        w1, w2 = WEIGHTS.get(spec.fc1[0], dt), WEIGHTS.get(spec.fc2[0], dt)
        ops.gemm(h2, w1, bias=spec.fc1[1], act=spec.act, aux_out=pre, out_t=f, tile_cfg=_rows_tile_cfg(M, w1, like, dt, act=True, aux_out=train, out_t=True))
        x2 = torch.empty(B, 1, D, device=like.device, dtype=torch.float32)
        ops.gemm(f, w2, bias=spec.fc2[1], resid=x1, out32=x2.view(B, D), tile_cfg=_rows_tile_cfg(M, w2, like, dt, out32=True, resid=True))
        if train:
            saved, ctx.layout = handoff.save_layout(x3.resid3 if x3 is not None else x, qkv, a, lse, x1, pre)
            ctx.save_for_backward(*saved)
            ctx.xshape = (B, N, D)
            ctx.spec = spec
            ctx.g3_out = dt == torch.bfloat16 and _g3_partner_feeds(x)
            ctx.cls_ok = False
            ctx.cls_fwd = True
        handoff.cls_rows_out(True)
        return x2

    @staticmethod
    def backward_cls(ctx, cg):
        compact = getattr(ctx, "cls_fwd", False)
        xin, qkv, a, lse, x1, pre = handoff.restore_layout(ctx.saved_tensors, ctx.layout)
        x3_in = isinstance(xin, Resid3)
        x = xin.lo if x3_in else xin
        spec = ctx.spec
        B, N, D = ctx.xshape
        M, dt = B * N, qkv.dtype
        F = pre.shape[1]
        dy = cg.rows32
        dy_t = dy if dt == torch.float32 else (cg.rows_t if cg.rows_t is not None else t_copy_of(dy, dt))
        pre_cls = pre if compact else ops.copy_rows(pre, N, _empty((B, F), dt, x))
        dpre = _empty((B, F), dt, x)
        ops.gemm(dy_t, WEIGHTS.get(spec.fc2[0], dt, transpose=True), dact=spec.act, aux_in=pre_cls, out_t=dpre)
        dh = _empty((B, D), dt, x)
        ops.gemm(dpre, WEIGHTS.get(spec.fc1[0], dt, transpose=True), out_t=dh)
        x1_cls = x1 if compact else ops.copy_rows(x1, N, _empty((B, D), torch.float32, x))
        dx1 = _empty((B, D), torch.float32, x)
        dx1_t = _empty((B, D), dt, x) if dt != torch.float32 else dx1
        ops.layernorm_bwd(dh, x1_cls, spec.ln2[0], spec.eps, dres=dy, dx32=dx1, dx_t=dx1_t if dt != torch.float32 else None)
        da = dh
        ops.gemm(dx1_t, WEIGHTS.get(spec.proj[0], dt, transpose=True), out_t=da)
        dqkv = _attn_act(M, 3 * D, dt, x, D)
        if ops.is_kb(dqkv):
            ops.attn_bwd_cls(qkv[:, :D], qkv[:, D:2 * D], qkv[:, 2 * D:], a, da, lse, dqkv, None, None, B, spec.heads, N, rows=compact)
        else:
            ops.attn_bwd_cls(qkv[:, :D], qkv[:, D:2 * D], qkv[:, 2 * D:], a, da, lse, dqkv[:, :D], dqkv[:, D:2 * D], dqkv[:, 2 * D:], B, spec.heads, N, rows=compact)
        dh1 = _empty((M, D), dt, x)
        ops.gemm(dqkv, WEIGHTS.get(spec.qkv[0], dt, transpose=True), out_t=dh1)
        xrows = xin if x3_in else x.view(M, D)
        if getattr(ctx, "g3_out", False):
            dx_t = _empty((M, D), dt, x)
            dlo = torch.empty(M, D, device=x.device, dtype=torch.int8)
            ops.layernorm_bwd_periodic(dh1, xrows, spec.ln1[0], spec.eps, dx1, N, dx_t=dx_t, dx_lo=dlo)
            return publish_grad3((B, N, D), x.device, dx_t, dlo), None
        dx = torch.empty(B, N, D, device=x.device, dtype=torch.float32)
        if dt == torch.float32:
            ops.layernorm_bwd_periodic(dh1, xrows, spec.ln1[0], spec.eps, dx1, N, dx32=dx.view(M, D))
            return dx, None
        dx_t = _empty((M, D), dt, x)
        ops.layernorm_bwd(dh1, xrows, spec.ln1[0], spec.eps, dres=ClsGrad(dx1, None, N).decode().view(M, D), dx32=dx.view(M, D), dx_t=dx_t)
        publish_t_copy(dx, dx_t)
        return dx, None

    @staticmethod
    def backward(ctx, dx2):
        if getattr(ctx, "cls_fwd", False):
            dx2 = dx2.contiguous()
            B, N, D = ctx.xshape
            dt = ctx.saved_tensors[-1].dtype
            return VitBlockFn.backward_cls(ctx, ClsGrad(dx2.view(B, D), t_copy_of(dx2, dt).view(B, D) if dt != torch.float32 else None, N))
        cg = cls_grad_of(dx2)
        if cg is not None:
            if getattr(ctx, "cls_ok", False):
                return VitBlockFn.backward_cls(ctx, cg)
            dx2 = cg.decode()
        g3 = grad3_of(dx2)
        xin, qkv, a, lse, x1, pre = handoff.restore_layout(ctx.saved_tensors, ctx.layout)
        x3_in, r3 = isinstance(xin, Resid3), isinstance(x1, Resid3)
        x = xin.lo if x3_in else xin
        spec = ctx.spec
        B, N, D = ctx.xshape
        M, dt = B * N, qkv.dtype
        F = pre.shape[1]
        if g3 is not None:
            dx2_t = g3.hi if ops.is_kb(g3.hi) else g3.hi.view(M, D)
            dres2 = Resid3(dx2_t, g3.lo)
        else:
            dx2 = dx2.contiguous()
            dx2_t = t_copy_of(dx2, dt, allow_kb=True)
            if not ops.is_kb(dx2_t):
                dx2_t = dx2_t.view(M, D)
            dres2 = dx2.view(M, D)
        g3_mode = g3 is not None or getattr(ctx, "g3_out", False)
        dpre = _act(M, F, dt, x, D)
        ops.gemm(dx2_t, WEIGHTS.get(spec.fc2[0], dt, transpose=True), dact=spec.act, aux_in=pre, out_t=dpre)
        dh = _empty((M, D), dt, x)
        ops.gemm(dpre, WEIGHTS.get(spec.fc1[0], dt, transpose=True), out_t=dh)
        del dpre
        if r3 or g3_mode:
            dx1_t = _empty((M, D), dt, x)
            dlo1 = torch.empty(M, D, device=x.device, dtype=torch.int8)
            ops.layernorm_bwd(dh, x1, spec.ln2[0], spec.eps, dres=dres2, dx_t=dx1_t, dx_lo=dlo1)
            dx1 = Resid3(dx1_t, dlo1)
        else:
            dx1 = torch.empty_like(x1)
            dx1_t = _empty((M, D), dt, x) if dt != torch.float32 else dx1
            ops.layernorm_bwd(dh, x1, spec.ln2[0], spec.eps, dres=dres2, dx32=dx1, dx_t=dx1_t if dt != torch.float32 else None)
        da = dh
        ops.gemm(dx1_t, WEIGHTS.get(spec.proj[0], dt, transpose=True), out_t=da)
        dqkv = _attn_act(M, 3 * D, dt, x, D) if D == 64 * spec.heads else _empty((M, 3 * D), dt, x)
        if ops.is_kb(dqkv):
            ops.attn_bwd(qkv[:, :D], qkv[:, D:2 * D], qkv[:, 2 * D:], a, da, lse, dqkv, None, None, B, spec.heads, N, mask=spec.mask)
        else:
            ops.attn_bwd(qkv[:, :D], qkv[:, D:2 * D], qkv[:, 2 * D:], a, da, lse, dqkv[:, :D], dqkv[:, D:2 * D], dqkv[:, 2 * D:], B, spec.heads, N, mask=spec.mask)
        ops.gemm(dqkv, WEIGHTS.get(spec.qkv[0], dt, transpose=True), out_t=da)
        dx_t = _empty((M, D), dt, x) if dt != torch.float32 else None
        xrows = xin if x3_in else x.view(M, D)
        if getattr(ctx, "g3_out", False):
            dlo = torch.empty(M, D, device=x.device, dtype=torch.int8)
            ops.layernorm_bwd(da, xrows, spec.ln1[0], spec.eps, dres=dx1, dx_t=dx_t, dx_lo=dlo)
            return publish_grad3((B, N, D), x.device, dx_t, dlo), None
        dx = torch.empty(B, N, D, device=x.device, dtype=torch.float32)
        ops.layernorm_bwd(da, xrows, spec.ln1[0], spec.eps, dres=dx1, dx32=dx.view(M, D), dx_t=dx_t)
        publish_t_copy(dx, dx_t)
        return dx, None


def vit_block(x, spec):
    return VitBlockFn.apply(x, spec)


class LnResidual:
    __slots__ = ("raw", "stats", "w", "b", "dim", "eps", "hi", "lo")

    def __init__(self, raw, stats, w, b, dim=None, eps=None, hi=None, lo=None):
        self.raw, self.stats, self.w, self.b = raw, stats, w, b
        self.dim, self.eps = dim, eps
        self.hi, self.lo = hi, lo

    def gemm_kw(self):
        if self.lo is not None:
            return dict(resid3=Resid3(self.hi, self.lo), resid_ln=(self.stats, self.w, self.b, self.dim, self.eps))
        if self.stats is None:
            return dict(resid=self.raw)
        if self.dim is None:
            return dict(resid=self.raw, resid_ln=(self.stats, self.w, self.b))
        return dict(resid=self.raw, resid_ln=(self.stats, self.w, self.b, self.dim, self.eps))


def _post_ln(raw, w, b, eps, x_t, stats_buf=None):
    if _STATE.get("text_ln_deferred", True):
        stats = stats_buf if stats_buf is not None else torch.empty(raw.shape[0], 2, device=raw.device, dtype=torch.float32)
        ops.layernorm_fwd(raw, w, b, eps, y_t=x_t, stats=stats)
        return LnResidual(raw, stats, w, b)
    ops.layernorm_fwd(raw, w, b, eps, y_t=x_t, y32=raw)
    return LnResidual(raw, None, w, b)


def post_ln_embed(e32, ln, x_t):
    return _post_ln(e32, ln.weight, ln.bias, ln.eps, x_t)


def _res_cls_rows(res, L, B, D, eps):
    rows = torch.empty(B, D, device=res.w.device, dtype=torch.float32)
    if res.lo is not None:
        ops.rows3_to_f32(res.hi, res.lo, L, rows)
    else:
        ops.copy_rows(res.raw.view(-1, D), L, rows)
        if res.stats is None:
            return rows
    ops.layernorm_fwd(rows, res.w, res.b, res.eps if res.eps is not None else eps, y32=rows)
    return rows


def post_ln_layer_cls_ok(x_t, heads, L, cu_seqlens=None):
    D = x_t.cols if ops.is_kb(x_t) else x_t.shape[1]
    return cu_seqlens is None and D == 64 * heads and 1 < L <= 288 and x_t.is_cuda and not (x_t.dtype != torch.float32 and _STATE.get("text_resid_t", False))

# ... 151 lines not shown
            Ep = (E + 63) // 64 * 64
            dfp = df.new_zeros(B, Ep)
            dfp[:, :E] = df
            df = dfp
            wt = WEIGHTS.get(w, hdt, transpose=not w_is_in_out, **({"pad_cols_to": Ep} if w_is_in_out else {"pad_rows_to": Ep}))
        else:
            wt = WEIGHTS.get(w, hdt, transpose=not w_is_in_out)
        ops.gemm(df, wt, out_t=dh)
        if hdt != dt:
            dh_t = _empty((B, D), dt, x)
            ops.cast(dh, dh_t)
            dh = dh_t
        if getattr(ctx, "cls_out", False):
            x_cls = ops.copy_rows(x.view(B * N, D), N, _empty((B, D), torch.float32, x))
            rows32 = _empty((B, D), torch.float32, x)
            rows_t = _empty((B, D), dt, x) if dt != torch.float32 else None
            ops.layernorm_bwd(dh, x_cls, ln_w, eps, dx32=rows32, dx_t=rows_t)
            return publish_cls_grad(x.shape, x.device, rows32, rows_t), None, None, None, None, None
        dx = torch.zeros_like(x)
        dx_t = torch.zeros(B * N, D, device=x.device, dtype=dt) if dt != torch.float32 else None
        ops.layernorm_bwd(dh, x, ln_w, eps, dx32=dx, dx_t=dx_t, rows=B, ldx=N * D)
        publish_t_copy(dx, dx_t)
        return dx, None, None, None, None, None


class LayerNormFn(torch.autograd.Function):

    @staticmethod
    def forward(ctx, x, w, b, eps):
        D = x.shape[-1]
        x2 = x.contiguous().view(-1, D)
        y = _empty(x2.shape, compute_dtype(), x)
        ops.layernorm_fwd(x2, w, b, eps, y_t=y)
        ctx.save_for_backward(x2, w)
        ctx.meta = (eps, x.shape)
        return y.view(x.shape)

    @staticmethod
    def backward(ctx, dy):
        x2, w = ctx.saved_tensors
        eps, shape = ctx.meta
        dx = torch.empty_like(x2)
        ops.layernorm_bwd(dy.contiguous().view(x2.shape), x2, w, eps, dx32=dx)
        return dx.view(shape), None, None, None


class AttentionFn(torch.autograd.Function):

    @staticmethod
    def forward(ctx, q, k, v, B, H, L, mask):
        kind, keylen = (mask[0], mask[1]) if isinstance(mask, tuple) else (mask, None)
        out = _empty((B * L, H * 64), q.dtype, q)
        need = any(ctx.needs_input_grad[:3])
        lse = torch.empty(B, H, L, device=q.device, dtype=torch.float32) if need else None
        ops.attn_fwd(q, k, v, out, B, H, L, lse=lse, mask=kind, keylen=keylen)
        if need:
            ctx.save_for_backward(q, k, v, out, lse)
            ctx.meta = (B, H, L, kind, keylen)
        return out

    @staticmethod
    def backward(ctx, dout):
        q, k, v, out, lse = ctx.saved_tensors
        B, H, L, kind, keylen = ctx.meta
        D = H * 64
        dqkv = _empty((B * L, 3 * D), q.dtype, q)
        ops.attn_bwd(q, k, v, out, dout.contiguous(), lse, dqkv[:, :D], dqkv[:, D:2 * D], dqkv[:, 2 * D:], B, H, L, mask=kind, keylen=keylen)
        return dqkv[:, :D], dqkv[:, D:2 * D], dqkv[:, 2 * D:], None, None, None, None


class MlpHalfFn(torch.autograd.Function):

    @staticmethod
    def forward(ctx, x1, spec):
        shape = x1.shape
        D = shape[-1]
        x1 = x1.contiguous().view(-1, D)
        M, dt = x1.shape[0], compute_dtype()
        train = ctx.needs_input_grad[0]
        h = _empty((M, D), dt, x1)
        ops.layernorm_fwd(x1, spec.ln2[0], spec.ln2[1], spec.eps, y_t=h)
        F = spec.fc1[0].shape[0]
        f = _empty((M, F), dt, x1)
        pre = _empty((M, F), dt, x1) if train else None
        ops.gemm(h, WEIGHTS.get(spec.fc1[0], dt), bias=spec.fc1[1], act=spec.act, aux_out=pre, out_t=f)
        x2 = torch.empty_like(x1)
        ops.gemm(f, WEIGHTS.get(spec.fc2[0], dt), bias=spec.fc2[1], resid=x1, out32=x2)
        if train:
            ctx.save_for_backward(x1, pre)
            ctx.meta = (spec, shape)
        return x2.view(shape)

    @staticmethod
    def backward(ctx, dx2):
        x1, pre = ctx.saved_tensors
        spec, shape = ctx.meta
        M, D = x1.shape
        dt = pre.dtype
        dx2 = dx2.contiguous().view(M, D)
        dx2_t = t_copy_of(dx2, dt)
        dpre = _empty(pre.shape, dt, x1)
        ops.gemm(dx2_t, WEIGHTS.get(spec.fc2[0], dt, transpose=True), dact=spec.act, aux_in=pre, out_t=dpre)
        dh = _empty((M, D), dt, x1)
        ops.gemm(dpre, WEIGHTS.get(spec.fc1[0], dt, transpose=True), out_t=dh)
        dx1 = torch.empty_like(x1)
        dx1_t = _empty((M, D), dt, x1) if dt != torch.float32 else None
        ops.layernorm_bwd(dh, x1, spec.ln2[0], spec.eps, dres=dx2, dx32=dx1, dx_t=dx1_t)
        publish_t_copy(dx1, dx1_t)
        return dx1.view(shape), None


LORA_PAD = 64


def _rank_pad(r):
    return max(LORA_PAD, (int(r) + LORA_PAD - 1) // LORA_PAD * LORA_PAD)


class LoraLinearFn(torch.autograd.Function):

    @staticmethod
    def forward(ctx, x, weight, bias, A, Bm, scaling, p_drop, resid32, direct=False):
        dt = x.dtype
        M, K = x.shape
        N = weight.shape[0]
        r = A.shape[0]
        y32 = torch.empty(M, N, device=x.device, dtype=torch.float32) if resid32 is not None else None
        y_t = _empty((M, N), dt, x) if resid32 is None else None
        kext = (r > 0 and ops.LORA_KEXT and dt == torch.bfloat16 and _rank_pad(r) == 64 and x.is_cuda and ops.KBLOCK_W and x.is_contiguous() and M >= 256
                and K % 32 == 0 and N % 8 == 0)
        if not kext:
            ops.gemm(x, WEIGHTS.get(weight, dt), bias=bias, resid=resid32, out32=y32, out_t=y_t)
        seed = 0
        xd = x
        t = None
        if r > 0:
            rp = _rank_pad(r)
            t = _empty((M, rp), dt, x)
            a_op = WEIGHTS.get(A, dt, pad_rows_to=rp)
            fuse = p_drop > 0 and dt == torch.bfloat16 and rp == 64 and x.is_cuda and x.is_contiguous() and 64 * (2 * K + 16) <= 160 * 1024 and K % 32 == 0
            regen = fuse and ops.LORA_REGEN_DROP and K % 64 == 0
            if p_drop > 0:
                seed = _next_seed()
                if not regen:
                    xd = torch.empty_like(x)
                if not fuse:
                    ops.dropout(x, xd, p_drop, seed)
            if fuse:
                ops.gemm(x, a_op.row, out_t=t, drop=("a", p_drop, seed, None if regen else xd))
            else:
                ops.gemm(xd, a_op, out_t=t)
            if kext:
                ops.gemm(x, WEIGHTS.get_lora_ext((weight,), (Bm,), scaling, dt, rp), bias=bias, resid=resid32, out32=y32, out_t=y_t, a2=(t, 0))
            else:
                bmat = WEIGHTS.get(Bm, dt, pad_cols_to=rp)
                if y32 is not None:
                    ops.gemm(t, bmat, alpha=scaling, resid=y32, out32=y32)
                else:
                    ops.gemm(t, bmat, alpha=scaling, resid_t=y_t, out_t=y_t)
        ctx.save_for_backward(xd, t if t is not None else x.new_empty(0), weight, A, Bm)
        ctx.meta = (scaling, p_drop, seed, r, bias is not None, resid32 is not None)
        ctx.regen = (p_drop, seed) if (r > 0 and regen) else None
        ctx.direct_params = (A, Bm, bias) if direct else None
        return y32 if y32 is not None else y_t

    @staticmethod
    def backward(ctx, dy):
        xd, t, weight, A, Bm = ctx.saved_tensors
        scaling, p_drop, seed, r, has_bias, has_resid = ctx.meta
        dt = xd.dtype
        M, K = xd.shape
        N = weight.shape[0]
        dy = dy.contiguous()
        dy_t = t_copy_of(dy, dt) if dy.dtype == torch.float32 else dy
        dx = _empty((M, K), dt, xd)
        ops.gemm(dy_t, WEIGHTS.get(weight, dt, transpose=True), out_t=dx)
        dA = dB = db = None
        pA, pB, pb = ctx.direct_params if ctx.direct_params is not None else (None, None, None)
        want_b = has_bias and ctx.needs_input_grad[2]
        direct = pA is not None and _is_flat_grad(pA) and _is_flat_grad(pB) and (not want_b or (pb is not None and _is_flat_grad(pb)))
        if want_b and not direct:
            db = torch.zeros(N, device=xd.device, dtype=torch.float32)
        gb = (pb.grad if direct else db) if want_b else None
        if r > 0:
            rp = _rank_pad(r)
# ... 916 lines not shown
```

nextgen-uia_amd/uia_hip/ops.py:

```python
import ctypes as C
from typing import NamedTuple

import torch

from . import _lib
from ._lib import AttnDesc, GemmDesc, LnLoraDesc, LoraRankDesc, MonaFusedDesc, MonaSpatialDesc, PackDesc, UiaError, WgradGroupDesc, check, lib

_ACT = {None: 0, "none": 0, "gelu": 1, "quick_gelu": 2, "relu": 3}

GEMM_PROFILE = None


EPI_BIAS, EPI_AUX_OUT, EPI_GELU, EPI_DGELU, EPI_RESID, EPI_RESIDT, EPI_OUT32, EPI_OUTT, EPI_RESID_LN, EPI_GENERIC = 1, 2, 4, 8, 16, 32, 64, 128, 256, -1
EPI_QUICK = 2048
EPI_ROWSUM, EPI_LNFOLD = 512, 1024
EPI_RESID_LO, EPI_OUT_LO = 4096, 8192
_SPECIALISED = {EPI_BIAS | EPI_RESID | EPI_OUT32, EPI_BIAS | EPI_RESIDT | EPI_OUT32, EPI_BIAS | EPI_RESID | EPI_RESID_LN | EPI_OUT32, EPI_OUTT, EPI_BIAS | EPI_OUTT, EPI_BIAS | EPI_GELU | EPI_OUTT, EPI_DGELU | EPI_OUTT,
                EPI_BIAS | EPI_GELU | EPI_AUX_OUT | EPI_OUTT,
                EPI_QUICK | EPI_BIAS | EPI_GELU | EPI_OUTT, EPI_QUICK | EPI_DGELU | EPI_OUTT, EPI_QUICK | EPI_BIAS | EPI_GELU | EPI_AUX_OUT | EPI_OUTT,
                EPI_BIAS | EPI_RESID | EPI_OUT32 | EPI_OUTT | EPI_ROWSUM, EPI_BIAS | EPI_RESID | EPI_RESID_LN | EPI_OUT32 | EPI_OUTT | EPI_ROWSUM,
                EPI_BIAS | EPI_OUTT | EPI_LNFOLD, EPI_BIAS | EPI_GELU | EPI_OUTT | EPI_LNFOLD, EPI_BIAS | EPI_GELU | EPI_AUX_OUT | EPI_OUTT | EPI_LNFOLD,
                EPI_QUICK | EPI_BIAS | EPI_GELU | EPI_OUTT | EPI_LNFOLD, EPI_QUICK | EPI_BIAS | EPI_GELU | EPI_AUX_OUT | EPI_OUTT | EPI_LNFOLD,
                EPI_BIAS | EPI_RESID_LO | EPI_RESID_LN | EPI_OUTT | EPI_OUT_LO | EPI_ROWSUM,
                EPI_BIAS | EPI_RESID | EPI_OUTT | EPI_OUT_LO | EPI_ROWSUM, EPI_BIAS | EPI_RESID_LO | EPI_OUT32,
                EPI_BIAS | EPI_RESID | EPI_RESID_LN | EPI_OUTT | EPI_OUT_LO | EPI_ROWSUM, EPI_BIAS | EPI_RESID_LO | EPI_RESID_LN | EPI_OUT32,
                EPI_BIAS | EPI_RESID_LO | EPI_OUT32 | EPI_OUTT | EPI_ROWSUM}

_QUAD_SPECIALISED = _SPECIALISED - {EPI_BIAS | EPI_RESIDT | EPI_OUT32, EPI_BIAS | EPI_RESID | EPI_RESID_LN | EPI_OUT32, EPI_BIAS | EPI_RESID | EPI_RESID_LN | EPI_OUT32 | EPI_OUTT | EPI_ROWSUM,
                                    EPI_BIAS | EPI_RESID | EPI_RESID_LN | EPI_OUTT | EPI_OUT_LO | EPI_ROWSUM, EPI_BIAS | EPI_RESID_LO | EPI_RESID_LN | EPI_OUT32,
                                    EPI_BIAS | EPI_RESID_LO | EPI_OUT32 | EPI_OUTT | EPI_ROWSUM}


def epi_mask_of(d):
    if d.alpha != 1.0 or d.out_group > 0 or d.resid_mod > 0:
        return EPI_GENERIC
    gl = (_ACT["gelu"], _ACT["quick_gelu"])
    if (d.act and d.act not in gl) or (d.dact and d.dact not in gl) or (d.act and d.dact and d.act != d.dact):
        return EPI_GENERIC
    quick = _ACT["quick_gelu"] in (d.act, d.dact)
    m = ((EPI_QUICK if quick else 0) | (EPI_BIAS if d.bias else 0) | (EPI_AUX_OUT if d.aux_out else 0) | (EPI_GELU if d.act else 0) | (EPI_DGELU if d.dact else 0) |
         (EPI_RESID if d.resid else 0) | (EPI_RESIDT if (d.residT and not d.resid_lo8) else 0) | (EPI_OUT32 if d.out32 else 0) | (EPI_OUTT if d.outT else 0) |
         (EPI_RESID_LN if ((d.resid or d.resid_lo8) and d.resid_ln_stats) else 0) | (EPI_ROWSUM if d.rowsum_out else 0) | (EPI_LNFOLD if d.lnfold_sums else 0) |
         (EPI_RESID_LO if d.resid_lo8 else 0) | (EPI_OUT_LO if d.out_lo8 else 0))
    return m


def auto_tile_cfg(M, N, K=None, esz=2, mask=EPI_GENERIC):
    if N <= 64:
        stream64 = N == 64 and M > 2048 and esz == 2 and K is not None and K % 32 == 0 and 64 * (2 * K + 16) <= 160 * 1024
        if stream64 and mask in (EPI_OUTT, EPI_BIAS | EPI_OUTT, EPI_GENERIC):
            return 16
        return 14 if (M > 2048 and esz == 2 and K is not None and K >= 1024) else 4
    if M <= 2048:
        return 21 if (esz == 4 and ((M + 127) // 128) * ((N + 127) // 128) < 64) else 3
    if K is not None and K * esz <= 128:
        return 14
    return 8


RING_CFGS = (8, 9, 10, 12, 13, 14, 24, 25, 26, 27, 28, 29)
PERSIST_STORE_ONLY = False
KBLOCK_W = True
K64_CFG14 = True
TILE_GROUP = {}
SHORT_K_WIDE_HALF_STASH = True
SHORT_K_WIDE_HALF_BYTES = 2048
SHORT_K_WIDE_HALF_N = 3072
HALF_HEIGHT_SHORT_K_ALWAYS = False
HALF_HEIGHT_SHORT_K = True
CHAINS = 1
TAIL_SPLIT = True
TAIL_SIDE_STREAM = True
MONA_PRE_FWD_T = True
MONA_PRE_BWD_DU = True
LN_LORA_DOWN = True
LORA_REGEN_DROP = True
LORA_RANK3 = True
QUAD = False
QUADV = False
RING5 = False
LORA_KEXT = True
TAIL_SPLIT_K = True
_SPLITK_WS = {}
_TRACE_GENERIC = {} if __import__("os").environ.get("UIA_TRACE_GENERIC") else None
_TAIL_SIDE = {}
_NCU = {}


def num_cus(device=None):
    dev = torch.cuda.current_device() if device is None else device
    if dev not in _NCU:
        _NCU[dev] = torch.cuda.get_device_properties(dev).multi_processor_count
    return _NCU[dev]


def big_tile_cfg(N, K, esz):
    if QUAD and esz == 2:
        return 25
    if QUADV and esz == 2:
        return QUADV if QUADV in (27, 29) else 27
    return 24 if (RING5 and esz == 2 and (K * esz >= 2048 or N >= 2304)) else 8


def tail_k_slices(rows, N, K, esz, ncu):
    tiles = -(-rows // 128) * -(-N // 256)
    kb = K * esz
    if not TAIL_SPLIT_K or esz != 2 or kb < 4096 or 4 * tiles > ncu:
        return 0
    s = min(ncu // tiles, kb // 1024, 16)
    return s if s >= 2 else 0


def splitk_workspace(floats, device):
    key = (device.index if device.index is not None else torch.cuda.current_device(), torch.cuda.current_stream(device).cuda_stream)
    t = _SPLITK_WS.get(key)
    if t is None or t.numel() < floats:
        t = _SPLITK_WS[key] = torch.zeros(max(floats, 1 << 20), device=device, dtype=torch.float32)
    return t


class _TailFork:

    def __init__(self, device):
# ... 132 lines not shown
        st = torch.cuda.current_stream()
        self.event = torch.cuda.Event()
        self.event.record(st)
        self.seen = {st.cuda_stream}

    def sync(self):
        rs = raw_stream()
        if rs not in self.seen:
            torch.cuda.current_stream().wait_event(self.event)
            self.seen.add(rs)


class PackedW:
    __slots__ = ("_row", "_kb", "ready", "kb_ready")

    def __init__(self, row, kb=None):
        self._row, self._kb = row, kb
        self.ready = Ready() if row.is_cuda else None
        self.kb_ready = self.ready

    def refreshed(self, ready):
        self.ready = self.kb_ready = ready

    @property
    def row(self):
        if self.ready is not None:
            self.ready.sync()
        return self._row

    @property
    def shape(self):
        return self._row.shape

    @property
    def dtype(self):
        return self._row.dtype

    @property
    def device(self):
        return self._row.device

    def kblocked(self):
        if self._kb is None:
            row = self.row
            N, K = row.shape
            g = 64 // row.element_size()
            self._kb = row.view(N, K // g, g).permute(1, 0, 2).contiguous()
            self.kb_ready = Ready() if row.is_cuda else None
        elif self.kb_ready is not None:
            self.kb_ready.sync()
        return self._kb


class ExtW:
    __slots__ = ("_kb", "N", "K", "K2", "ready", "__weakref__")

    def __init__(self, kb, N, K, K2):
        self._kb, self.N, self.K, self.K2 = kb, N, K, K2
        self.ready = Ready() if kb.is_cuda else None

    @property
    def kb(self):
        if self.ready is not None:
            self.ready.sync()
        return self._kb

    @property
    def device(self):
        return self._kb.device


class RawDest:
    __slots__ = ("view",)

    def __init__(self, view):
        self.view = view


def gemm_kernel_name(cfg, mask, dtype):
    m = mask if mask in _SPECIALISED else EPI_GENERIC
    tn, tc = ("bf16", "DF16b") if dtype == torch.bfloat16 else ("float", "f")
    mi = lambda v: f"Li{v}E" if v >= 0 else f"Lin{-v}E"
    if cfg == 12:
        return f"gemm_tn_persist_kernel<{tn},{m}>", f"gemm_tn_persist_kernelI{tc}{mi(m)}E"
    if cfg in (8, 13, 14, 24):
        bm, nbuf = (256, 4) if cfg == 8 else ((256, 5) if cfg == 24 else ((128, 4) if cfg == 13 else (128, 3)))
        return f"gemm_tn_ring_kernel<{tn},{bm},256,2,4,64,{nbuf},{m}>", "gemm_tn_ring_kernelI" + tc + "".join(mi(v) for v in (bm, 256, 2, 4, 64, nbuf, m, 0)) + "Lb0ELb0EE"
    if cfg in (25, 26):
        mq = m if (cfg == 25 and m in _QUAD_SPECIALISED) else EPI_GENERIC
        return f"gemm_tn_quad_kernel<{mq},false>", f"gemm_tn_quad_kernelI{mi(mq)}Lb0EE"
    if cfg == 29:
        mq = m if m in _QUAD_SPECIALISED else EPI_GENERIC
        return f"gemm_tn_quadvp_kernel<{mq}>", f"gemm_tn_quadvp_kernelI{mi(mq)}E"
    if cfg in (27, 28):
        mq = m if (m in _QUAD_SPECIALISED and (cfg == 27 or m == EPI_OUTT)) else EPI_GENERIC
        return f"gemm_tn_quadv_kernel<{mq},{cfg - 25},0>", f"gemm_tn_quadv_kernelI{mi(mq)}{mi(cfg - 25)}Li0EE"
    if cfg == 16:
        return "gemm_skinny64_kernel", "gemm_skinny64_kernel"
    if cfg == 23:
        return "gemm_wide64_kernel", "gemm_wide64_kernel"
    shape = {1: (256, 256, 2, 4), 2: (256, 128, 4, 2), 3: (128, 128, 2, 2), 4: (256, 64, 4, 1), 5: (128, 64, 2, 1), 21: (32, 64, 2, 2)}.get(cfg)
    if shape:
        return f"gemm_tn_kernel<{tn},{','.join(map(str, shape))}>", "gemm_tn_kernelI" + tc + "".join(mi(v) for v in shape) + "E"
    return f"tile cfg {cfg}", f"cfg{cfg}"


def _code(dt):
    if dt == torch.bfloat16:
        return _lib.BF16
    if dt == torch.float32:
        return _lib.F32
    raise UiaError(f"unsupported operand dtype {dt}")


def _p(t):
    if t is None:
        return None
    if not t.is_cuda:
        raise UiaError("uia ops need CUDA/HIP tensors: there is no CPU fallback for the hot path")
    return t.data_ptr()


_HIP_OK = []


def raw_stream():
    return torch._C._cuda_getCurrentRawStream(torch._C._cuda_getDevice())


def _stream():
    if not _HIP_OK:
        if not torch.cuda.is_available():
            raise UiaError("uia ops need an MI355X (HIP) device: there is no CPU fallback for the hot path")
        _HIP_OK.append(True)
    return raw_stream()


def _dense(t, name, dtypes, numel=None, align=1):
    if not isinstance(t, torch.Tensor):
        raise UiaError(f"{name}: a tensor is required, got {type(t).__name__}")
    if t.dtype not in dtypes:
        raise UiaError(f"{name}: dtype {t.dtype}, expected {' or '.join(str(d) for d in dtypes)}")
    if not t.is_contiguous():
        raise UiaError(f"{name}: must be contiguous (shape {tuple(t.shape)}, stride {t.stride()})")
    if numel is not None and t.numel() != numel:
        raise UiaError(f"{name}: {t.numel()} elements (shape {tuple(t.shape)}), expected {numel}")
    if align == "v4":
        align = 4 * t.element_size()
    if t.data_ptr() % align:
        raise UiaError(f"{name}: data pointer not aligned to {align} bytes")
    return t


def _require(cond, msg):
    if not cond:
        raise UiaError(msg)


_F32, _FT = (torch.float32,), (torch.bfloat16, torch.float32)


def _rowmajor(t, name):
    if t.dim() != 2 or t.stride(1) != 1:
        raise UiaError(f"{name} must be a 2-D row-major tensor (got shape {tuple(t.shape)}, stride {t.stride()})")
    return t.stride(0)


class Launch(NamedTuple):
    lo: int
    hi: int
    tile_cfg: int
    base: int
    w_kblocked: bool
    side: bool
    scratch: int


def plan_gemm(M, N, K, esz, ncu, tile_cfg=0, *, whole=False, ext=False, packed=False, on_device=True, out_group=0, resid_mod=0, drop=None, alpha=1.0,
              a_kb=False, out_t_kb=False, act=False, aux_out=False, out_t=False, out32=False, resid=False, resid_t=False, rowsum=False, ln=False):
    auto = 0 if (ext or tile_cfg & 255) else auto_tile_cfg(M, N, K, esz)

    def launch(lo, hi, word, side=False, scratch=0):
        base = word & 255
        if ext:
            if not base:
                base = 8 if hi - lo > 2048 else 13
                word |= base
        elif not base:
            base = auto
            if (base == 14 and esz == 2 and K == 64 and N % 64 == 0 and N * 144 <= 160 * 1024 and not (a_kb or out_t_kb or act or aux_out or rowsum or ln)
                    and out_group == 0 and resid_mod == 0 and drop in (None, "acc")
                    and ((out_t and not out32 and not resid and (resid_t or drop is not None)) or (out32 and not out_t and not resid_t and (resid or drop is not None)))):
                base = 23
            elif base == 8:
                base = big_tile_cfg(N, K, esz)
                word |= base
        if PERSIST_STORE_ONLY and base == 8 and not (resid or resid_t or out32 or rowsum) and out_group == 0 and alpha == 1.0 and K * esz >= 1024:
            base, word = 12, (word & ~255) | 12
        if TILE_GROUP and N in TILE_GROUP and (word >> 8) == 0 and base in RING_CFGS:
            word |= int(TILE_GROUP[N]) << 8
        return Launch(lo, hi, word, base, bool(ext or (packed and KBLOCK_W and base in RING_CFGS and on_device)), side, scratch)

    m_main = M
    if whole or not on_device:
        pass
    elif ext:
        if TAIL_SPLIT and tile_cfg == 0 and M > 2048:
            m_main = tail_split_rows(M, N, ncu)
    else:
        if not K64_CFG14 and tile_cfg == 0 and auto == 14:
            tile_cfg = 8
        if TAIL_SPLIT and tile_cfg == 0 and out_group == 0 and resid_mod == 0 and drop is None and auto == 8:
            m_main = tail_split_rows(M, N, ncu)
            if SHORT_K_WIDE_HALF_N and N >= SHORT_K_WIDE_HALF_N and K * esz <= SHORT_K_WIDE_HALF_BYTES and esz == 2 and (SHORT_K_WIDE_HALF_STASH or not aux_out):
                tile_cfg, m_main = 14, M
            if (m_main < M or HALF_HEIGHT_SHORT_K_ALWAYS) and HALF_HEIGHT_SHORT_K and CHAINS <= 1 and N <= 768 and K * esz <= 1536:
                tile_cfg, m_main = 14, M
    if m_main == M:
        return [launch(0, M, tile_cfg)]
    side = small_tail(M - m_main, N, ncu)
    if CHAINS > 1 and not side and not ext:
        return [launch(0, M, tile_cfg)]
    slices = 0 if ext else tail_k_slices(M - m_main, N, K, esz, ncu)
    if slices:
        floats = -(-(M - m_main) // 128) * -(-N // 256) * 128 * 256
        tail = [launch(m_main, M, 13 | slices << 16 | phase << 22, side, floats) for phase in (1, 2)]
    else:
        tail = [launch(m_main, M, 13, side)]
    main = launch(0, m_main, 8 if ext else big_tile_cfg(N, K, esz))
    return tail + [main] if side else [main] + tail


def _plan_facts(a, w, act, dact, aux_out, out_group, resid_mod, drop, alpha, out_t, out32, resid, resid_t, rowsum, lnfold, resid_ln):
    return dict(ext=isinstance(w, ExtW), packed=isinstance(w, PackedW), on_device=a.is_cuda, out_group=out_group, resid_mod=resid_mod,
                drop=None if drop is None else drop[0], alpha=alpha, a_kb=is_kb(a), out_t_kb=is_kb(out_t), act=act is not None or dact is not None,
                aux_out=aux_out is not None, out_t=out_t is not None, out32=out32 is not None, resid=resid is not None, resid_t=resid_t is not None,
                rowsum=rowsum is not None, ln=lnfold is not None or resid_ln is not None)


def _cut(t, lo, hi, heads=1):
    if t is None:
        return None
    if isinstance(t, tuple):
        return tuple(_cut(x, lo, hi) for x in t[:heads]) + tuple(t[heads:])
    if is_kb(t):
        return t.row_range(lo, hi)
    return t[lo:hi] if t.dim() < 3 else t[:, lo:hi]


def gemm(a, w, *, bias=None, act=None, dact=None, aux_in=None, aux_out=None, resid=None, resid_mod=0, resid_row_off=0,
         resid_t=None, out_group=0, out_t=None, out32=None, alpha=1.0, tile_cfg=0, resid_ln=None, rowsum=None, lnfold=None, drop=None, a2=None,
         resid3=None, out_lo=None):
    if (resid3 is not None or out_lo is not None) and (isinstance(w, ExtW) or resid_mod or out_group or (a.t.dtype if is_kb(a) else a.dtype) != torch.bfloat16):
        raise UiaError("gemm: three-byte tensors (resid3 / out_lo) need bf16 operands and a plain epilogue (no row remapping, no K extension)")
    if isinstance(w, ExtW):
        if a2 is None or is_kb(a) or a.dtype != torch.bfloat16 or a.shape[1] != w.K - w.K2 or resid_mod or out_group or drop is not None:
            raise UiaError("gemm: an ExtW weight needs a2 = (t, group_cols), a row-major bf16 `a` of K - K2 columns and a plain epilogue")
        t2, gcols = a2
        M, N, K = a.shape[0], w.N, w.K
        if t2.dtype != a.dtype or t2.shape[-1] != w.K2 or t2.shape[-2] != M or t2.stride(-1) != 1 or t2.stride(-2) != w.K2 or (t2.dim() == 3 and t2.shape[0] * gcols != w.N):
            raise UiaError(f"gemm: a2 operand {tuple(t2.shape)} does not match [groups, {M}, {w.K2}] with {w.N} columns in groups of {gcols}")
    else:
        M, (N, K) = (a.rows if is_kb(a) else a.shape[0]), (w.row if isinstance(w, PackedW) else w).shape
    plan = plan_gemm(M, N, K, a.element_size(), num_cus(a.device.index) if a.is_cuda else 0, tile_cfg,
                     **_plan_facts(a, w, act, dact, aux_out, out_group, resid_mod, drop, alpha, out_t, out32, resid, resid_t, rowsum, lnfold, resid_ln))
    if len(plan) == 1:
        _gemm_one(a, w, bias=bias, act=act, dact=dact, aux_in=aux_in, aux_out=aux_out, resid=resid, resid_mod=resid_mod, resid_row_off=resid_row_off,
                  resid_t=resid_t, out_group=out_group, out_t=out_t, out32=out32, alpha=alpha, resid_ln=resid_ln, rowsum=rowsum, lnfold=lnfold, drop=drop,
                  a2=a2, resid3=resid3, out_lo=out_lo, launch=plan[0])
        return

    def run(launches):
        ws = None
        try:
            for L in launches:
                if L.scratch and ws is None:
                    ws = splitk_workspace(L.scratch, a.device)
                lo, hi = L.lo, L.hi
                _gemm_one(_cut(a, lo, hi), w, bias=bias, act=act, dact=dact, aux_in=_cut(aux_in, lo, hi), aux_out=_cut(aux_out, lo, hi), resid=_cut(resid, lo, hi),
                          resid_t=_cut(resid_t, lo, hi), out_t=_cut(out_t, lo, hi), out32=_cut(out32, lo, hi), alpha=alpha, resid_ln=_cut(resid_ln, lo, hi),
                          rowsum=_cut(rowsum, lo, hi), lnfold=_cut(lnfold, lo, hi), splitk_ws=ws if L.scratch else None, a2=_cut(a2, lo, hi),
                          resid3=_cut(resid3, lo, hi, 2), out_lo=_cut(out_lo, lo, hi), launch=L)
        except Exception:
            if ws is not None:
                drop_splitk_workspace(a.device)
            raise

    side = [L for L in plan if L.side]
    if side:
        fork = _TailFork(a.device)
        with fork:
            run(side)
        run([L for L in plan if not L.side])
        fork.join()
    else:
        run(plan)


def _plane(t, name, M, N, dtype, rows_checked=True):
    if is_kb(t):
        rows, cols, plane = _kb_dims(t, f"gemm {name}")
        if rows < M or cols != N or t.t.dtype != dtype:
            raise UiaError(f"gemm {name} (K-blocked {tuple(t.t.shape)} {t.t.dtype}) does not hold the [{M}, {N}] {dtype} plane")
        return t.t, N, plane
    if t.dtype != dtype or t.dim() != 2 or t.shape[1] < N or (rows_checked and t.shape[0] < M):
        raise UiaError(f"gemm {name} is {tuple(t.shape)} {t.dtype}: it does not hold the [{M}, {N}] {dtype} plane")
    return t, _rowmajor(t, name), 0


def _gemm_one(a, w, *, bias=None, act=None, dact=None, aux_in=None, aux_out=None, resid=None, resid_mod=0, resid_row_off=0,
              resid_t=None, out_group=0, out_t=None, out32=None, alpha=1.0, tile_cfg=0, resid_ln=None, rowsum=None, lnfold=None, drop=None, splitk_ws=None, a2=None,
              resid3=None, out_lo=None, launch=None):
    d = GemmDesc()
    if splitk_ws is not None:
        d.splitk_ws = _p(splitk_ws)
    ext = w if isinstance(w, ExtW) else None
    if ext is not None:
        t2, gcols = a2
        d.A2, d.lda2, d.K2 = t2.data_ptr(), t2.stride(-2), ext.K2
        d.a2_group_cols, d.a2_group_stride = (gcols, t2.stride(0)) if t2.dim() == 3 else (0, 0)
    if drop is not None:
        d.drop_where, d.drop_p, d.drop_seed = {"a": 1, "acc": 2}[drop[0]], float(drop[1]), int(drop[2]) & 0xFFFFFFFFFFFFFFFF
        if len(drop) > 3 and drop[3] is not None:
            xo = drop[3]
            if drop[0] != "a" or xo.dtype != a.dtype or xo.shape != a.shape or xo.stride() != a.stride():
                raise UiaError("gemm drop: a_drop_out must have a's dtype, shape and strides")
            d.a_drop_out = _p(xo)
    packed = w if isinstance(w, PackedW) else None
    if ext is not None:
        d.lda, d.ldw, d.M, d.K, d.N = _rowmajor(a, "a"), ext.K, a.shape[0], ext.K, ext.N
        d.A = _p(a)
    else:
        wrow = packed.row if packed is not None else w
        d.ldw = _rowmajor(wrow, "w")
        if is_kb(a):
            d.M, d.K, d.a_kb_rows = _kb_dims(a, "gemm a")
            d.lda = d.K
        else:
            d.lda = _rowmajor(a, "a")
            d.M, d.K = a.shape[0], a.shape[1]
        if a.dtype != wrow.dtype or d.K != wrow.shape[1]:
            raise UiaError(f"gemm operand mismatch: a {(d.M, d.K)} {a.dtype}, w {tuple(wrow.shape)} {wrow.dtype}")
        d.A = _p(a.t if is_kb(a) else a)
        d.N = wrow.shape[0]
    esz = a.element_size()
    if launch is None:
        launch = plan_gemm(d.M, d.N, d.K, esz, 0, tile_cfg, whole=True,
                           **_plan_facts(a, w, act, dact, aux_out, out_group, resid_mod, drop, alpha, out_t, out32, resid, resid_t, rowsum, lnfold, resid_ln))[0]
    tile_cfg, base_cfg = launch.tile_cfg, launch.base
    d.W, d.w_kblocked = (_p(ext.kb if ext is not None else packed.kblocked()), 1) if launch.w_kblocked else (_p(wrow), 0)
    d.alpha = alpha
    d.act, d.dact = _ACT[act], _ACT[dact]
    if bias is not None:
        assert bias.dtype == torch.float32 and bias.numel() == d.N
        d.bias = _p(bias)
    for name, t, want in (("aux_in", aux_in, a.dtype), ("aux_out", aux_out, a.dtype), ("resid_t", resid_t, a.dtype),
                          ("resid", resid, torch.float32), ("out32", out32, torch.float32)):
        if t is not None and t.dtype != want:
            raise UiaError(f"gemm {name} must be {want}, got {t.dtype}")
    for name, t in (("aux_in", aux_in), ("aux_out", aux_out), ("resid_t", resid_t), ("out32", out32)):
        if t is not None and (t.dim() != 2 or t.shape[1] < d.N or (t.shape[0] < d.M and out_group == 0)):
            raise UiaError(f"gemm {name} is {tuple(t.shape)}: too small for the [{d.M}, {d.N}] result")
    if resid is not None and resid_mod == 0 and out_group == 0 and (resid.dim() != 2 or resid.shape[1] < d.N or resid.shape[0] < d.M):
        raise UiaError(f"gemm resid is {tuple(resid.shape)}: too small for the [{d.M}, {d.N}] result")
    if aux_in is not None:
        d.aux_in, d.ldaux_in = _p(aux_in), _rowmajor(aux_in, "aux_in")
    if aux_out is not None:
        d.aux_out, d.ldaux_out = _p(aux_out), _rowmajor(aux_out, "aux_out")
    if resid is not None:
        d.resid, d.ldr = _p(resid), _rowmajor(resid, "resid")
    d.resid_mod, d.resid_row_off, d.out_group = resid_mod, resid_row_off, out_group
    if resid_ln is not None:
        st, lw, lb = resid_ln[:3]
        if len(resid_ln) > 3:
            d.resid_ln_dim, d.resid_ln_eps = int(resid_ln[3]), float(resid_ln[4])
        if (resid is None and resid3 is None) or resid_mod or out_group:
            raise UiaError("gemm resid_ln needs a plain fp32 resid or a three-byte resid3 (no row remapping)")
        want_st = torch.int64 if len(resid_ln) > 3 else torch.float32
        if not (st.dtype == want_st and lw.dtype == lb.dtype == torch.float32 and st.is_contiguous() and st.numel() >= 2 * d.M and lw.numel() >= d.N and lb.numel() >= d.N):
            raise UiaError(f"gemm resid_ln: stats {tuple(st.shape)} / weight {tuple(lw.shape)} / bias {tuple(lb.shape)} do not cover [{d.M}, {d.N}]")
        d.resid_ln_stats, d.resid_ln_w, d.resid_ln_b = _p(st), _p(lw), _p(lb)
    if rowsum is not None:
        if not (rowsum.dtype == torch.int64 and rowsum.is_contiguous() and rowsum.numel() >= 2 * d.M) or out_group:
            raise UiaError(f"gemm rowsum must be a contiguous int64 [{d.M}, 2] tensor (no row remapping), got {tuple(rowsum.shape)} {rowsum.dtype}")
        d.rowsum_out = _p(rowsum)
    if lnfold is not None:
        sm, cs, dim, eps = lnfold
        if not (sm.dtype == torch.int64 and cs.dtype == torch.float32 and sm.is_contiguous() and cs.is_contiguous() and sm.numel() >= 2 * d.M and cs.numel() >= d.N) or alpha != 1.0:
            raise UiaError(f"gemm lnfold: sums {tuple(sm.shape)} {sm.dtype} / colsum {tuple(cs.shape)} do not cover [{d.M}, {d.N}] (int64 row sums, fp32 colsum, contiguous, alpha == 1)")
        d.lnfold_sums, d.lnfold_colsum, d.lnfold_dim, d.lnfold_eps = _p(sm), _p(cs), int(dim), float(eps)
    if (rowsum is not None or lnfold is not None) and a.is_cuda:
        d.ln_flag, d.ln_flag_limit = _p(ln_flag(a.device)), LN_FLAG_LIMIT
    if resid_t is not None:
        d.residT, d.ldrT = _p(resid_t), _rowmajor(resid_t, "resid_t")
    if resid3 is not None:
        if resid is not None or resid_t is not None:
            raise UiaError("gemm: resid3 replaces resid / resid_t")
        t, d.ldrT, d.residT_kb_rows = _plane(resid3[0], "resid3 hi plane", d.M, d.N, torch.bfloat16)
        d.residT = _p(t)
        t, d.ld_resid_lo, d.resid_lo_kb_rows = _plane(resid3[1], "resid3 low bytes", d.M, d.N, torch.int8)
        d.resid_lo8 = _p(t)
    if out_lo is not None:
        if out_t is None:
            raise UiaError("gemm out_lo needs out_t (the hi plane)")
        t, d.ld_out_lo, d.out_lo_kb_rows = _plane(out_lo, "out_lo", d.M, d.N, torch.int8)
        d.out_lo8 = _p(t)
    if out_t is not None:
        if out_group and is_kb(out_t):
            raise UiaError(f"gemm out_t (K-blocked {tuple(out_t.t.shape)}) does not hold the [{d.M}, {d.N}] result of a row-remapping launch")
        t, d.ldo, d.outT_kb_rows = _plane(out_t, "out_t", d.M, d.N, a.dtype, not out_group)
        d.outT = _p(t)
    if out32 is not None:
        d.out32, d.ldo32 = _p(out32), _rowmajor(out32, "out32")
    if GEMM_PROFILE is not None:
        e0, e1 = torch.cuda.Event(enable_timing=True), torch.cuda.Event(enable_timing=True)
        e0.record()
        check(lib().uia_gemm(_stream(), _code(a.dtype), C.byref(d), tile_cfg), "uia_gemm")
        e1.record()
        nbytes = esz * (d.M * d.K + d.N * d.K) + d.M * d.N * (esz * sum(t is not None for t in (aux_in, aux_out, resid_t, out_t))
                                                             + 4 * sum(t is not None for t in (resid, out32)) + 3 * (resid3 is not None) + 1 * (out_lo is not None))
        mask = epi_mask_of(d)
        if not (tile_cfg & 255) and base_cfg != 23:
            base_cfg = auto_tile_cfg(d.M, d.N, d.K, esz, mask)
        GEMM_PROFILE.append((e0, e1, d.M, d.N, d.K, a.dtype, base_cfg, nbytes, mask))
        return
    if _TRACE_GENERIC is not None:
        mask = epi_mask_of(d)
        if mask not in _SPECIALISED and d.M > 2048:
            _TRACE_GENERIC[(mask, d.M, d.N, d.K, base_cfg)] = _TRACE_GENERIC.get((mask, d.M, d.N, d.K, base_cfg), 0) + 1
    check(lib().uia_gemm(_stream(), _code(a.dtype), C.byref(d), tile_cfg), "uia_gemm")


def three_byte_to_float(hi, lo):
    h = hi.t.permute(1, 0, 2).reshape(hi.rows, hi.cols) if is_kb(hi) else hi
    lo = lo.t.permute(1, 0, 2).reshape(lo.rows, lo.cols) if is_kb(lo) else lo
    h = h[:lo.shape[0], :lo.shape[1]]
    bits = (h.contiguous().view(torch.int16).to(torch.int32) << 16) + (lo.to(torch.int32) << 8)
    return bits.view(torch.float32)


def float_to_three_byte(x):
    hi = x.bfloat16()
    xb = x.contiguous().view(torch.int32).to(torch.int64) & 0xFFFFFFFF
    hb = hi.contiguous().view(torch.int16).to(torch.int64) & 0xFFFF
    d = ((xb + 0x80) >> 8) - (hb << 8)
    return hi, d.clamp(-127, 127).to(torch.int8)


def wgrad(a, b, dw, dbias=None, alpha=1.0, drop=None):
    lda, ldb = _rowmajor(a, "a"), _rowmajor(b, "b")
    assert a.dtype == b.dtype and a.shape[0] == b.shape[0] and dw.dtype == torch.float32 and dw.is_contiguous() and dw.dim() == 2
    I, J = a.shape[1], b.shape[1]
    if drop is not None:
        p, seed = drop
        if dbias is not None or a.dtype != torch.bfloat16 or ldb != J:
            raise UiaError("wgrad(drop=...): bf16, no bias, and b must be the whole dropped tensor (contiguous rows)")
        check(lib().uia_wgrad_drop(_stream(), _code(a.dtype), a.shape[0], I, J, _p(a), lda, _p(b), ldb, alpha, _p(dw), dw.shape[1], dw.shape[0], dw.shape[1],
                                   float(p), int(seed) & 0xFFFFFFFFFFFFFFFF, J, 0), "uia_wgrad_drop")
        return
    if tuple(dw.shape) == (I, J):
        check(lib().uia_wgrad(_stream(), _code(a.dtype), a.shape[0], I, J, _p(a), lda, _p(b), ldb, alpha, _p(dw), _p(dbias)), "uia_wgrad")
        return
    assert dw.shape[0] <= I and dw.shape[1] <= J and (dbias is None or dbias.numel() >= dw.shape[0])
    check(lib().uia_wgrad_ex(_stream(), _code(a.dtype), a.shape[0], I, J, _p(a), lda, _p(b), ldb, alpha, _p(dw), dw.shape[1], dw.shape[0], dw.shape[1],
                             _p(dbias)), "uia_wgrad_ex")


LORA_WGRAD_GROUP = True


def wgrad_group(a_list, b_list, dw_list, dbias_list=None, alpha=1.0, drop=None):
    n = len(a_list)
    a0, b0, w0 = a_list[0], b_list[0], dw_list[0]
    if not (1 <= n <= 4 and len(b_list) == n and len(dw_list) == n and a0.dtype == torch.bfloat16):
        raise UiaError("wgrad_group: 1..4 bf16 problems")
    lda, ldb = _rowmajor(a0, "a"), _rowmajor(b0, "b")
    M, I, J = a0.shape[0], a0.shape[1], b0.shape[1]
    d = WgradGroupDesc()
    d.n, d.M, d.I, d.J, d.lda, d.ldb, d.ldw = n, M, I, J, lda, ldb, w0.shape[1]
    d.i_valid, d.j_valid, d.alpha = w0.shape[0], w0.shape[1], alpha
    for g in range(n):
        a, b, w = a_list[g], b_list[g], dw_list[g]
        if (a.dtype != torch.bfloat16 or b.dtype != torch.bfloat16 or tuple(a.shape) != (M, I) or tuple(b.shape) != (M, J) or _rowmajor(a, "a") != lda or _rowmajor(b, "b") != ldb
                or w.dtype != torch.float32 or not w.is_contiguous() or w.shape != w0.shape or w.shape[0] > I or w.shape[1] > J):
            raise UiaError(f"wgrad_group: problem {g} does not have the shape / strides / dtypes of problem 0")
        d.A[g], d.B[g], d.dW[g] = a.data_ptr(), b.data_ptr(), w.data_ptr()
        db = dbias_list[g] if dbias_list is not None else None
        if db is not None:
            assert db.dtype == torch.float32 and db.numel() >= w.shape[0]
            d.dbias_A[g] = db.data_ptr()
    if drop is not None:
        p_, seeds = drop
        if ldb != J or (dbias_list is not None and any(x is not None for x in dbias_list)):
            raise UiaError("wgrad_group(drop=...): no bias, and each b must be the whole dropped tensor (contiguous rows)")
        d.drop_p, d.drop_ld, d.drop_col0 = float(p_), J, 0
        for g in range(n):
            d.drop_seed[g] = int(seeds[g]) & 0xFFFFFFFFFFFFFFFF
    check(lib().uia_wgrad_group(_stream(), _code(a0.dtype), C.byref(d)), "uia_wgrad_group")


def _attn_desc(q, k, v, out, lse, B, H, L, mask, keylen, scale, dh=None):
    d = AttnDesc()
# ... 1552 lines not shown
```

Before: 6847.

## Stash quantized GELU derivative as uint8 instead of bf16 pre-activation

The fc1 forward GEMM epilogue now computes the GELU/QuickGELU derivative and stores it as one uint8 code per element (scale 1/192, zero point 25) instead of stashing the bf16 pre-activation. The backward fc2 dgrad epilogue decodes the byte and multiplies, so it no longer re-evaluates the derivative. This halves the MLP activation stash traffic for both the write and the read and removes derivative math from backward. In exchange the gradient is quantized to 8 bits with clamping, which changes numerics. It is on by default for bf16 training and adds new specialised epilogue instantiations.

```diff
diff --git a/include/uia_hip.h b/include/uia_hip.h
--- a/include/uia_hip.h
+++ b/include/uia_hip.h
@@ -8,7 +8,8 @@
 #endif
 
 enum { UIA_F32 = 0, UIA_BF16 = 1 };
-enum { UIA_ACT_NONE = 0, UIA_ACT_GELU = 1, UIA_ACT_QUICKGELU = 2, UIA_ACT_RELU = 3 };
+enum { UIA_ACT_NONE = 0, UIA_ACT_GELU = 1, UIA_ACT_QUICKGELU = 2, UIA_ACT_RELU = 3,
+       UIA_ACT_GELU_DBYTE = 4, UIA_ACT_QUICKGELU_DBYTE = 5 };
 enum { UIA_MASK_NONE = 0, UIA_MASK_CAUSAL = 1, UIA_MASK_KEYPAD = 2 };
 enum { UIA_MONA_BASELINE = 0, UIA_MONA_NOISE_AWARE = 1, UIA_MONA_FREQ_ENHANCED = 2, UIA_MONA_HYBRID = 3 };
 
diff --git a/nextgen-uia_amd/csrc/gemm.hip b/nextgen-uia_amd/csrc/gemm.hip
--- a/nextgen-uia_amd/csrc/gemm.hip
+++ b/nextgen-uia_amd/csrc/gemm.hip
@@ -832,6 +832,12 @@
             UIA_EPI_CASE(EPI_BIAS | EPI_GELU | EPI_AUX_OUT | EPI_OUTT | EPI_LNFOLD);
             UIA_EPI_CASE(EPI_QUICK | EPI_BIAS | EPI_GELU | EPI_OUTT | EPI_LNFOLD);
             UIA_EPI_CASE(EPI_QUICK | EPI_BIAS | EPI_GELU | EPI_AUX_OUT | EPI_OUTT | EPI_LNFOLD);
+            UIA_EPI_CASE(EPI_DBYTE | EPI_BIAS | EPI_GELU | EPI_AUX_OUT | EPI_OUTT | EPI_LNFOLD);
+            UIA_EPI_CASE(EPI_DBYTE | EPI_BIAS | EPI_GELU | EPI_AUX_OUT | EPI_OUTT);
+            UIA_EPI_CASE(EPI_DBYTE | EPI_DGELU | EPI_OUTT);
+            UIA_EPI_CASE(EPI_DBYTE | EPI_QUICK | EPI_BIAS | EPI_GELU | EPI_AUX_OUT | EPI_OUTT | EPI_LNFOLD);
+            UIA_EPI_CASE(EPI_DBYTE | EPI_QUICK | EPI_BIAS | EPI_GELU | EPI_AUX_OUT | EPI_OUTT);
+            UIA_EPI_CASE(EPI_DBYTE | EPI_QUICK | EPI_DGELU | EPI_OUTT);
 #undef UIA_EPI_CASE
             default: break;
         }
@@ -1218,8 +1224,11 @@
                   "uia_gemm: out_lo8 needs bf16, outT as the hi plane, 8-byte aligned rows of at least N bytes and no row remapping");
     UIA_CHECK_ARG(!p.bias || (uintptr_t)p.bias % 16 == 0, "uia_gemm: bias alignment");
     UIA_CHECK_ARG(!p.dact || p.aux_in, "uia_gemm: dact needs aux_in");
-    UIA_CHECK_ARG(!p.aux_in || (p.ldaux_in % 8 == 0 && (uintptr_t)p.aux_in % 16 == 0), "uia_gemm: aux_in alignment");
-    UIA_CHECK_ARG(!p.aux_out || (p.ldaux_out % 8 == 0 && (uintptr_t)p.aux_out % 16 == 0), "uia_gemm: aux_out alignment");
+    UIA_CHECK_ARG(p.act >= UIA_ACT_NONE && p.act <= UIA_ACT_QUICKGELU_DBYTE && p.dact >= UIA_ACT_NONE && p.dact <= UIA_ACT_QUICKGELU_DBYTE, "uia_gemm: unknown activation code act=%d dact=%d", p.act, p.dact);
+    UIA_CHECK_ARG(!(act_is_dbyte(p.act) || act_is_dbyte(p.dact)) || dtype == UIA_BF16, "uia_gemm: the derivative-byte activation codes are for bf16 launches");
+    UIA_CHECK_ARG(!act_is_dbyte(p.act) || p.aux_out, "uia_gemm: a derivative-byte act needs aux_out (the uint8 plane)");
+    UIA_CHECK_ARG(!p.aux_in || (p.ldaux_in % 8 == 0 && (uintptr_t)p.aux_in % (act_is_dbyte(p.dact) ? 8 : 16) == 0), "uia_gemm: aux_in alignment");
+    UIA_CHECK_ARG(!p.aux_out || (p.ldaux_out % 8 == 0 && (uintptr_t)p.aux_out % (act_is_dbyte(p.act) ? 8 : 16) == 0), "uia_gemm: aux_out alignment");
     UIA_CHECK_ARG(p.resid_mod == 0 || p.resid, "uia_gemm: resid_mod without resid");
     UIA_CHECK_ARG(!p.resid_ln_stats || ((p.resid || p.resid_lo8) && p.resid_ln_w && p.resid_ln_b), "uia_gemm: resid_ln_stats needs resid (or residT + resid_lo8), resid_ln_w and resid_ln_b");
     UIA_CHECK_ARG(!p.resid_ln_stats || ((uintptr_t)p.resid_ln_stats % 8 == 0 && (uintptr_t)p.resid_ln_w % 16 == 0 && (uintptr_t)p.resid_ln_b % 16 == 0),
diff --git a/nextgen-uia_amd/csrc/gemm_epilogue.h b/nextgen-uia_amd/csrc/gemm_epilogue.h
--- a/nextgen-uia_amd/csrc/gemm_epilogue.h
+++ b/nextgen-uia_amd/csrc/gemm_epilogue.h
@@ -89,6 +89,34 @@
         default: return 1.0f;
     }
 }
+__host__ __device__ __forceinline__ int act_base(int act) { return act >= UIA_ACT_GELU_DBYTE ? act - (UIA_ACT_GELU_DBYTE - UIA_ACT_GELU) : act; }
+__host__ __device__ __forceinline__ bool act_is_dbyte(int act) { return act >= UIA_ACT_GELU_DBYTE; }
+template <bool FAST>
+__device__ __forceinline__ void act_deriv8(const float (&a)[8], float (&d)[8], int act) {
+    if (FAST && act == UIA_ACT_GELU) {
+#pragma unroll
+        for (int e = 0; e < 8; e += 2) {
+            const f32x2 x = {a[e], a[e + 1]}, g = dgelu_poly2(x);
+            d[e] = g[0];
+            d[e + 1] = g[1];
+        }
+    } else {
+#pragma unroll
+        for (int e = 0; e < 8; ++e) d[e] = apply_dact<FAST>(a[e], act);
+    }
+}
+template <bool FAST>
+__device__ __forceinline__ void dact_byte_store8(void* aux_out, size_t off, const float (&v)[8], int act) {
+    float d[8];
+    act_deriv8<FAST>(v, d, act);
+    *(uint2*)((unsigned char*)aux_out + off) = dact_byte_encode8(d);
+}
+__device__ __forceinline__ void dact_byte_mul8(float (&v)[8], uint2 codes) {
+    float g[8];
+    dact_byte_decode8(codes, g);
+#pragma unroll
+    for (int e = 0; e < 8; ++e) v[e] *= g[e];
+}
 
 __device__ __forceinline__ void glds16(const char* gsrc, char* lds_wave_base) {
     __builtin_amdgcn_global_load_lds((const __attribute__((address_space(1))) void*)gsrc,
@@ -154,6 +182,7 @@
     const T* aux_in = (const T*)p.aux_in;
     T* aux_out = (T*)p.aux_out;
     const T* residT = (const T*)p.residT;
+    const int act = act_base(p.act), dact = act_base(p.dact);
 #pragma unroll
     for (int i = 0; i < MT; ++i) {
         const int m = m0 + wm * WTM + 16 * i + li;
@@ -182,14 +211,19 @@
 #pragma unroll
                 for (int e = 0; e < 8; ++e) v[e] += b[e];
             }
-            if (aux_out) store8(aux_out + orow * p.ldaux_out + n, v);
-            if (p.act) {
-                apply_act8<sizeof(T) == 2>(v, p.act);
-            }
-            if (p.dact) {
+            if (aux_out) {
+                if (act_is_dbyte(p.act)) dact_byte_store8<sizeof(T) == 2>(p.aux_out, orow * p.ldaux_out + n, v, act);
+                else store8(aux_out + orow * p.ldaux_out + n, v);
+            }
+            if (act) {
+                apply_act8<sizeof(T) == 2>(v, act);
+            }
+            if (act_is_dbyte(p.dact)) {
+                dact_byte_mul8(v, *(const uint2*)((const unsigned char*)p.aux_in + orow * p.ldaux_in + n));
+            } else if (dact) {
                 float a[8];
                 load8(aux_in + orow * p.ldaux_in + n, a);
-                apply_dact8<sizeof(T) == 2>(v, a, p.dact);
+                apply_dact8<sizeof(T) == 2>(v, a, dact);
             }
             if (p.drop_where == 2) {
                 const uint32_t keep = dropout_keep8(p.drop_seed, (uint32_t)(((size_t)m * (size_t)p.N + (size_t)n) >> 3), dropout_thresh16(p.drop_p));
@@ -246,6 +280,7 @@
              EPI_QUICK = 2048,
              EPI_RESID_LO = 4096,
              EPI_OUT_LO = 8192,
+             EPI_DBYTE = 16384,
              EPI_GENERIC = -1 };
 
 template <typename T, int MT, int NT, int WTM, int WTN, int EPI = EPI_GENERIC, bool PATCH16 = false, int WCOLS = 4>
@@ -263,8 +298,10 @@
     const bool f_outT = GEN ? p.outT != nullptr : (EPI & EPI_OUTT) != 0;
     const bool f_rowsum = GEN ? p.rowsum_out != nullptr : (EPI & EPI_ROWSUM) != 0;
     const bool f_lnfold = GEN ? p.lnfold_sums != nullptr : (EPI & EPI_LNFOLD) != 0;
-    const int act = GEN ? p.act : ((EPI & EPI_GELU) ? ((EPI & EPI_QUICK) ? UIA_ACT_QUICKGELU : UIA_ACT_GELU) : UIA_ACT_NONE);
-    const int dact = GEN ? p.dact : ((EPI & EPI_DGELU) ? ((EPI & EPI_QUICK) ? UIA_ACT_QUICKGELU : UIA_ACT_GELU) : UIA_ACT_NONE);
+    const int act = GEN ? act_base(p.act) : ((EPI & EPI_GELU) ? ((EPI & EPI_QUICK) ? UIA_ACT_QUICKGELU : UIA_ACT_GELU) : UIA_ACT_NONE);
+    const int dact = GEN ? act_base(p.dact) : ((EPI & EPI_DGELU) ? ((EPI & EPI_QUICK) ? UIA_ACT_QUICKGELU : UIA_ACT_GELU) : UIA_ACT_NONE);
+    const bool f_abyte = GEN ? act_is_dbyte(p.act) : (EPI & EPI_DBYTE) != 0;
+    const bool f_dbyte = GEN ? act_is_dbyte(p.dact) : (EPI & EPI_DBYTE) != 0;
     using EP = EpiPatch<MT, WTN>;
     constexpr int LDW = EP::LDW, GPP = EP::GPP, ROWS = EP::ROWS;
     constexpr int LPR = WTN / 8;
@@ -317,7 +354,7 @@
     }
 
     auto apply = [&](const f32x4& lo, const f32x4& hi, int m, const bf16x8* pre_aux = nullptr, const f32x4* pre_res = nullptr,
-                     const bf16x8* pre_rt = nullptr, float* os1 = nullptr, float* os2 = nullptr, const uint2* pre_lo = nullptr) {
+                     const bf16x8* pre_rt = nullptr, float* os1 = nullptr, float* os2 = nullptr, const uint2* pre_lo = nullptr, const uint2* pre_ab = nullptr) {
         const bool ok = m < p.M && col_ok;
         if (!f_rowsum && !ok) return;
         float v[8] = {lo[0], lo[1], lo[2], lo[3], hi[0], hi[1], hi[2], hi[3]};
@@ -343,9 +380,14 @@
 #pragma unroll
             for (int e = 0; e < 8; ++e) v[e] += bias[e];
         }
-        if (f_aux_out && UIA_EPI_STORES) store8(aux_out + orow * p.ldaux_out + n, v);
+        if (f_aux_out && UIA_EPI_STORES) {
+            if (f_abyte) dact_byte_store8<sizeof(T) == 2>(p.aux_out, orow * p.ldaux_out + n, v, act);
+            else store8(aux_out + orow * p.ldaux_out + n, v);
+        }
         if (act) apply_act8<sizeof(T) == 2>(v, act);
-        if (dact && UIA_EPI_LOADS) {
+        if (dact && f_dbyte && UIA_EPI_LOADS) {
+            dact_byte_mul8(v, pre_ab ? *pre_ab : *(const uint2*)((const unsigned char*)p.aux_in + orow * p.ldaux_in + n));
+        } else if (dact && UIA_EPI_LOADS) {
             float a[8];
             if (pre_aux) {
 #pragma unroll
@@ -580,10 +622,11 @@
             }
         } else
         if constexpr (PIPE && NPASS % 2 == 0) {
-            constexpr bool H_AUX = (EPI & EPI_DGELU) != 0, H_RES = (EPI & EPI_RESID) != 0, H_LO = (EPI & EPI_RESID_LO) != 0, H_RT = (EPI & EPI_RESIDT) != 0 || H_LO,
+            constexpr bool H_AB = (EPI & EPI_DGELU) != 0 && (EPI & EPI_DBYTE) != 0, H_AUX = (EPI & EPI_DGELU) != 0 && !H_AB, H_RES = (EPI & EPI_RESID) != 0, H_LO = (EPI & EPI_RESID_LO) != 0, H_RT = (EPI & EPI_RESIDT) != 0 || H_LO,
                            H_SUM = (EPI & EPI_ROWSUM) != 0;
             constexpr int CH = NPASS / 2, NCH = 2 * NPH;
             bf16x8 pa[2][H_AUX ? CH : 1];
+            uint2 pab[2][H_AB ? CH : 1];
             f32x4 pr[2][H_RES ? 2 * CH : 1];
             bf16x8 prt[2][H_RT ? CH : 1];
             uint2 plo[2][H_LO ? CH : 1];
@@ -597,6 +640,7 @@
                     const int m = mrow + (c * CH + q) * RPP;
                     const size_t mc = (size_t)(m < p.M ? m : p.M - 1);
                     if constexpr (H_AUX) pa[set][q] = *(const bf16x8*)((const bf16_t*)p.aux_in + mc * p.ldaux_in + nc);
+                    if constexpr (H_AB) pab[set][q] = *(const uint2*)((const unsigned char*)p.aux_in + mc * p.ldaux_in + nc);
                     if constexpr (H_RES) { const float* src = p.resid + mc * p.ldr + nc; pr[set][2 * q] = *(const f32x4*)src; pr[set][2 * q + 1] = *(const f32x4*)(src + 4); }
                     if constexpr (H_LO) {
                         const bf16_t* hp = p.residT_kb_rows ? (const bf16_t*)p.residT + ((size_t)(nc / 32) * (size_t)p.residT_kb_rows + mc) * 32 + (nc % 32)
@@ -624,7 +668,8 @@
                     const int row = ((c & 1) * CH + q) * RPP + rr;
                     const f32x4 lo = *(const f32x4*)(stg + row * LDW + rc), hi = *(const f32x4*)(stg + row * LDW + rc + 4);
                     apply(lo, hi, mrow + (c * CH + q) * RPP, H_AUX ? &pa[set][q] : nullptr, H_RES ? &pr[set][2 * q] : nullptr, H_RT ? &prt[set][q] : nullptr,
-                          H_SUM ? &rs1[c * CH + q] : nullptr, H_SUM ? &rs2[c * CH + q] : nullptr, H_LO ? &plo[set][q] : nullptr);
+                          H_SUM ? &rs1[c * CH + q] : nullptr, H_SUM ? &rs2[c * CH + q] : nullptr, H_LO ? &plo[set][q] : nullptr,
+                          H_AB ? &pab[set][q] : nullptr);
                 }
                 if (c + 2 < NCH) issue(c + 2, set);
                 if ((c & 1) == 1) __builtin_amdgcn_wave_barrier();
@@ -685,10 +730,11 @@
 
 inline int epi_mask_of(const UiaGemmParams& p) {
     if (p.alpha != 1.0f || p.out_group > 0 || p.resid_mod > 0 || p.drop_where == 2) return EPI_GENERIC;
-    const bool quick = p.act == UIA_ACT_QUICKGELU || p.dact == UIA_ACT_QUICKGELU;
-    if ((p.act && p.act != UIA_ACT_GELU && p.act != UIA_ACT_QUICKGELU) || (p.dact && p.dact != UIA_ACT_GELU && p.dact != UIA_ACT_QUICKGELU) ||
+    const int act = act_base(p.act), dact = act_base(p.dact);
+    const bool quick = act == UIA_ACT_QUICKGELU || dact == UIA_ACT_QUICKGELU;
+    if ((act && act != UIA_ACT_GELU && act != UIA_ACT_QUICKGELU) || (dact && dact != UIA_ACT_GELU && dact != UIA_ACT_QUICKGELU) ||
         (p.act && p.dact && p.act != p.dact)) return EPI_GENERIC;
-    return (quick ? EPI_QUICK : 0) | (p.bias ? EPI_BIAS : 0) | (p.aux_out ? EPI_AUX_OUT : 0) | (p.act ? EPI_GELU : 0) | (p.dact ? EPI_DGELU : 0) | (p.resid ? EPI_RESID : 0) |
+    return ((act_is_dbyte(p.act) || act_is_dbyte(p.dact)) ? EPI_DBYTE : 0) | (quick ? EPI_QUICK : 0) | (p.bias ? EPI_BIAS : 0) | (p.aux_out ? EPI_AUX_OUT : 0) | (p.act ? EPI_GELU : 0) | (p.dact ? EPI_DGELU : 0) | (p.resid ? EPI_RESID : 0) |
            ((p.resid && p.resid_ln_stats) ? EPI_RESID_LN : 0) | (p.rowsum_out ? EPI_ROWSUM : 0) | (p.lnfold_sums ? EPI_LNFOLD : 0) |
            ((p.residT && !p.resid_lo8) ? EPI_RESIDT : 0) | (p.out32 ? EPI_OUT32 : 0) | (p.outT ? EPI_OUTT : 0) |
            (p.resid_lo8 ? EPI_RESID_LO : 0) | ((p.resid_lo8 && p.resid_ln_stats) ? EPI_RESID_LN : 0) | (p.out_lo8 ? EPI_OUT_LO : 0);
diff --git a/nextgen-uia_amd/csrc/uia_common.h b/nextgen-uia_amd/csrc/uia_common.h
--- a/nextgen-uia_amd/csrc/uia_common.h
+++ b/nextgen-uia_amd/csrc/uia_common.h
@@ -81,6 +81,21 @@
     return r;
 }
 
+constexpr float DACT_BYTE_SCALE = 192.0f, DACT_BYTE_ZERO = 25.0f, DACT_BYTE_STEP = 1.0f / 192.0f;
+__device__ __forceinline__ uint2 dact_byte_encode8(const float (&g)[8]) {
+    unsigned w[2] = {0u, 0u};
+#pragma unroll
+    for (int e = 0; e < 8; ++e) {
+        const float t = __builtin_amdgcn_fmed3f(__builtin_rintf(g[e] * DACT_BYTE_SCALE) + DACT_BYTE_ZERO, 0.0f, 255.0f);
+        w[e >> 2] = __builtin_amdgcn_cvt_pk_u8_f32(t, e & 3, w[e >> 2]);
+    }
+    return uint2{w[0], w[1]};
+}
+__device__ __forceinline__ void dact_byte_decode8(uint2 c, float (&g)[8]) {
+#pragma unroll
+    for (int e = 0; e < 8; ++e) g[e] = ((float)(((e < 4 ? c.x : c.y) >> (8 * (e & 3))) & 0xFFu) - DACT_BYTE_ZERO) * DACT_BYTE_STEP;
+}
+
 #endif
 
 inline int uia_num_cus() {
diff --git a/nextgen-uia_amd/uia_hip/functional.py b/nextgen-uia_amd/uia_hip/functional.py
--- a/nextgen-uia_amd/uia_hip/functional.py
+++ b/nextgen-uia_amd/uia_hip/functional.py
@@ -39,6 +39,22 @@
 
 def set_text_resid3(flag):
     _STATE["text_resid3"] = bool(flag)
+
+
+def set_dact_byte(flag):
+    _STATE["dact_byte"] = bool(flag)
+
+
+def _mlp_stash(M, F, dt, like, act, train):
+    if not train:
+        return None, act
+    if dt == torch.bfloat16 and _STATE.get("dact_byte", True) and act in ("gelu", "quick_gelu"):
+        return torch.empty((M, F), device=like.device, dtype=torch.uint8), ops.dact_byte_of(act)
+    return _empty((M, F), dt, like), act
+
+
+def _mlp_dact(stash, act):
+    return ops.dact_byte_of(act) if stash.dtype == torch.uint8 else act
 
 
 def set_ln_fold(flag):
@@ -638,7 +654,7 @@
             ops.attn_fwd(qkv[:, :D], qkv[:, D:2 * D], qkv[:, 2 * D:], a, B, spec.heads, N, lse=lse, mask=spec.mask)
         F = spec.fc1[0].shape[0]
         f = _act(M, F, dt, like, D)
-        pre = _empty((M, F), dt, like) if train else None
+        pre, act1 = _mlp_stash(M, F, dt, like, spec.act, train)
         r3 = fold and _STATE.get("block_resid3", False) and dt == torch.bfloat16 and M > 2048
         x1 = None if r3 else torch.empty(M, D, device=like.device, dtype=torch.float32)
         lo1 = torch.empty(M, D, device=like.device, dtype=torch.int8) if r3 else None
@@ -648,12 +664,12 @@
             resx = dict(resid3=x3.resid3) if x3 is not None else dict(resid=x2d)
             ops.gemm(a, WEIGHTS.get(spec.proj[0], dt), bias=spec.proj[1], out32=x1, out_t=h1, out_lo=lo1, rowsum=sums1, **resx)
             w1, c1, b1 = WEIGHTS.get_lnfold(spec.fc1[0], spec.fc1[1], spec.ln2[0], spec.ln2[1], dt)
-            ops.gemm(h1, w1, bias=b1, act=spec.act, aux_out=pre, out_t=f, lnfold=(sums1, c1, D, spec.eps))
+            ops.gemm(h1, w1, bias=b1, act=act1, aux_out=pre, out_t=f, lnfold=(sums1, c1, D, spec.eps))
         else:
             ops.gemm(a, WEIGHTS.get(spec.proj[0], dt), bias=spec.proj[1], resid=x2d, out32=x1)
             h1 = _as_act(h1, M, D, dt, 0)
             ops.layernorm_fwd(x1, spec.ln2[0], spec.ln2[1], spec.eps, y_t=h1)
-            ops.gemm(h1, WEIGHTS.get(spec.fc1[0], dt), bias=spec.fc1[1], act=spec.act, aux_out=pre, out_t=f)
+            ops.gemm(h1, WEIGHTS.get(spec.fc1[0], dt), bias=spec.fc1[1], act=act1, aux_out=pre, out_t=f)
         x2 = torch.empty(B, N, D, device=like.device, dtype=torch.float32)
         res1 = dict(resid3=Resid3(h1, lo1)) if r3 else dict(resid=x1)
         if fold and spec.publish_out:
@@ -692,9 +708,9 @@
         ops.layernorm_fwd(x1, spec.ln2[0], spec.ln2[1], spec.eps, y_t=h2)
         F = spec.fc1[0].shape[0]
         f = _empty((B, F), dt, like)
-        pre = _empty((B, F), dt, like) if train else None
+        pre, act1 = _mlp_stash(B, F, dt, like, spec.act, train)
         w1, w2 = WEIGHTS.get(spec.fc1[0], dt), WEIGHTS.get(spec.fc2[0], dt)
-        ops.gemm(h2, w1, bias=spec.fc1[1], act=spec.act, aux_out=pre, out_t=f, tile_cfg=_rows_tile_cfg(M, w1, like, dt, act=True, aux_out=train, out_t=True))
+        ops.gemm(h2, w1, bias=spec.fc1[1], act=act1, aux_out=pre, out_t=f, tile_cfg=_rows_tile_cfg(M, w1, like, dt, act=True, aux_out=train, out_t=True))
         x2 = torch.empty(B, 1, D, device=like.device, dtype=torch.float32)
         ops.gemm(f, w2, bias=spec.fc2[1], resid=x1, out32=x2.view(B, D), tile_cfg=_rows_tile_cfg(M, w2, like, dt, out32=True, resid=True))
         if train:
@@ -705,6 +721,7 @@
             ctx.g3_out = dt == torch.bfloat16 and _g3_partner_feeds(x)
             ctx.cls_ok = False
             ctx.cls_fwd = True
+            ctx.dt = dt
         handoff.cls_rows_out(True)
         return x2
 
@@ -720,9 +737,9 @@
         F = pre.shape[1]
         dy = cg.rows32
         dy_t = dy if dt == torch.float32 else (cg.rows_t if cg.rows_t is not None else t_copy_of(dy, dt))
-        pre_cls = pre if compact else ops.copy_rows(pre, N, _empty((B, F), dt, x))
+        pre_cls = pre if compact else ops.copy_rows(pre, N, _empty((B, F), pre.dtype, x))
         dpre = _empty((B, F), dt, x)
-        ops.gemm(dy_t, WEIGHTS.get(spec.fc2[0], dt, transpose=True), dact=spec.act, aux_in=pre_cls, out_t=dpre)
+        ops.gemm(dy_t, WEIGHTS.get(spec.fc2[0], dt, transpose=True), dact=_mlp_dact(pre, spec.act), aux_in=pre_cls, out_t=dpre)
         dh = _empty((B, D), dt, x)
         ops.gemm(dpre, WEIGHTS.get(spec.fc1[0], dt, transpose=True), out_t=dh)
         x1_cls = x1 if compact else ops.copy_rows(x1, N, _empty((B, D), torch.float32, x))
@@ -758,7 +775,7 @@
         if getattr(ctx, "cls_fwd", False):
             dx2 = dx2.contiguous()
             B, N, D = ctx.xshape
-            dt = ctx.saved_tensors[-1].dtype
+            dt = ctx.dt
             return VitBlockFn.backward_cls(ctx, ClsGrad(dx2.view(B, D), t_copy_of(dx2, dt).view(B, D) if dt != torch.float32 else None, N))
         cg = cls_grad_of(dx2)
         if cg is not None:
@@ -784,7 +801,7 @@
             dres2 = dx2.view(M, D)
         g3_mode = g3 is not None or getattr(ctx, "g3_out", False)
         dpre = _act(M, F, dt, x, D)
-        ops.gemm(dx2_t, WEIGHTS.get(spec.fc2[0], dt, transpose=True), dact=spec.act, aux_in=pre, out_t=dpre)
+        ops.gemm(dx2_t, WEIGHTS.get(spec.fc2[0], dt, transpose=True), dact=_mlp_dact(pre, spec.act), aux_in=pre, out_t=dpre)
         dh = _empty((M, D), dt, x)
         ops.gemm(dpre, WEIGHTS.get(spec.fc1[0], dt, transpose=True), out_t=dh)
         del dpre
@@ -1102,25 +1119,24 @@
         ops.layernorm_fwd(x1, spec.ln2[0], spec.ln2[1], spec.eps, y_t=h)
         F = spec.fc1[0].shape[0]
         f = _empty((M, F), dt, x1)
-        pre = _empty((M, F), dt, x1) if train else None
-        ops.gemm(h, WEIGHTS.get(spec.fc1[0], dt), bias=spec.fc1[1], act=spec.act, aux_out=pre, out_t=f)
+        pre, act1 = _mlp_stash(M, F, dt, x1, spec.act, train)
+        ops.gemm(h, WEIGHTS.get(spec.fc1[0], dt), bias=spec.fc1[1], act=act1, aux_out=pre, out_t=f)
         x2 = torch.empty_like(x1)
         ops.gemm(f, WEIGHTS.get(spec.fc2[0], dt), bias=spec.fc2[1], resid=x1, out32=x2)
         if train:
             ctx.save_for_backward(x1, pre)
-            ctx.meta = (spec, shape)
+            ctx.meta = (spec, shape, dt)
         return x2.view(shape)
 
     @staticmethod
     def backward(ctx, dx2):
         x1, pre = ctx.saved_tensors
-        spec, shape = ctx.meta
+        spec, shape, dt = ctx.meta
         M, D = x1.shape
-        dt = pre.dtype
         dx2 = dx2.contiguous().view(M, D)
         dx2_t = t_copy_of(dx2, dt)
         dpre = _empty(pre.shape, dt, x1)
-        ops.gemm(dx2_t, WEIGHTS.get(spec.fc2[0], dt, transpose=True), dact=spec.act, aux_in=pre, out_t=dpre)
+        ops.gemm(dx2_t, WEIGHTS.get(spec.fc2[0], dt, transpose=True), dact=_mlp_dact(pre, spec.act), aux_in=pre, out_t=dpre)
         dh = _empty((M, D), dt, x1)
         ops.gemm(dpre, WEIGHTS.get(spec.fc1[0], dt, transpose=True), out_t=dh)
         dx1 = torch.empty_like(x1)
diff --git a/nextgen-uia_amd/uia_hip/ops.py b/nextgen-uia_amd/uia_hip/ops.py
--- a/nextgen-uia_amd/uia_hip/ops.py
+++ b/nextgen-uia_amd/uia_hip/ops.py
@@ -6,7 +6,20 @@
 from . import _lib
 from ._lib import AttnDesc, GemmDesc, LnLoraDesc, LoraRankDesc, MonaFusedDesc, MonaSpatialDesc, PackDesc, UiaError, WgradGroupDesc, check, lib
 
-_ACT = {None: 0, "none": 0, "gelu": 1, "quick_gelu": 2, "relu": 3}
+_ACT = {None: 0, "none": 0, "gelu": 1, "quick_gelu": 2, "relu": 3,
+        "gelu_dbyte": 4, "quick_gelu_dbyte": 5}
+_DBYTE = {"gelu": "gelu_dbyte", "quick_gelu": "quick_gelu_dbyte"}
+DACT_BYTE_SCALE, DACT_BYTE_ZERO = 192.0, 25.0
+
+
+def dact_byte_of(act):
+    if act not in _DBYTE:
+        raise UiaError(f"no derivative-byte form of activation {act!r}")
+    return _DBYTE[act]
+
+
+def dact_byte_decode(codes):
+    return (codes.to(torch.float32) - DACT_BYTE_ZERO) * torch.tensor(1.0 / DACT_BYTE_SCALE, dtype=torch.float32, device=codes.device)
 
 GEMM_PROFILE = None
 
@@ -15,6 +28,7 @@
 EPI_QUICK = 2048
 EPI_ROWSUM, EPI_LNFOLD = 512, 1024
 EPI_RESID_LO, EPI_OUT_LO = 4096, 8192
+EPI_DBYTE = 16384
 _SPECIALISED = {EPI_BIAS | EPI_RESID | EPI_OUT32, EPI_BIAS | EPI_RESIDT | EPI_OUT32, EPI_BIAS | EPI_RESID | EPI_RESID_LN | EPI_OUT32, EPI_OUTT, EPI_BIAS | EPI_OUTT, EPI_BIAS | EPI_GELU | EPI_OUTT, EPI_DGELU | EPI_OUTT,
                 EPI_BIAS | EPI_GELU | EPI_AUX_OUT | EPI_OUTT,
                 EPI_QUICK | EPI_BIAS | EPI_GELU | EPI_OUTT, EPI_QUICK | EPI_DGELU | EPI_OUTT, EPI_QUICK | EPI_BIAS | EPI_GELU | EPI_AUX_OUT | EPI_OUTT,
@@ -25,20 +39,27 @@
                 EPI_BIAS | EPI_RESID | EPI_OUTT | EPI_OUT_LO | EPI_ROWSUM, EPI_BIAS | EPI_RESID_LO | EPI_OUT32,
                 EPI_BIAS | EPI_RESID | EPI_RESID_LN | EPI_OUTT | EPI_OUT_LO | EPI_ROWSUM, EPI_BIAS | EPI_RESID_LO | EPI_RESID_LN | EPI_OUT32,
                 EPI_BIAS | EPI_RESID_LO | EPI_OUT32 | EPI_OUTT | EPI_ROWSUM}
+_DBYTE_MASKS = {q | m for q in (0, EPI_QUICK) for m in (EPI_DBYTE | EPI_BIAS | EPI_GELU | EPI_AUX_OUT | EPI_OUTT | EPI_LNFOLD, EPI_DBYTE | EPI_BIAS | EPI_GELU | EPI_AUX_OUT | EPI_OUTT,
+                                                        EPI_DBYTE | EPI_DGELU | EPI_OUTT)}
+_SPECIALISED |= _DBYTE_MASKS
+_PERSIST_SPECIALISED = {EPI_BIAS | EPI_RESID | EPI_OUT32, EPI_BIAS | EPI_RESIDT | EPI_OUT32, EPI_OUTT, EPI_BIAS | EPI_OUTT, EPI_BIAS | EPI_GELU | EPI_OUTT, EPI_DGELU | EPI_OUTT,
+                        EPI_BIAS | EPI_GELU | EPI_AUX_OUT | EPI_OUTT, EPI_BIAS | EPI_OUTT | EPI_LNFOLD, EPI_BIAS | EPI_GELU | EPI_OUTT | EPI_LNFOLD,
+                        EPI_BIAS | EPI_GELU | EPI_AUX_OUT | EPI_OUTT | EPI_LNFOLD}
 
 _QUAD_SPECIALISED = _SPECIALISED - {EPI_BIAS | EPI_RESIDT | EPI_OUT32, EPI_BIAS | EPI_RESID | EPI_RESID_LN | EPI_OUT32, EPI_BIAS | EPI_RESID | EPI_RESID_LN | EPI_OUT32 | EPI_OUTT | EPI_ROWSUM,
                                     EPI_BIAS | EPI_RESID | EPI_RESID_LN | EPI_OUTT | EPI_OUT_LO | EPI_ROWSUM, EPI_BIAS | EPI_RESID_LO | EPI_RESID_LN | EPI_OUT32,
-                                    EPI_BIAS | EPI_RESID_LO | EPI_OUT32 | EPI_OUTT | EPI_ROWSUM}
+                                    EPI_BIAS | EPI_RESID_LO | EPI_OUT32 | EPI_OUTT | EPI_ROWSUM} - _DBYTE_MASKS
 
 
 def epi_mask_of(d):
     if d.alpha != 1.0 or d.out_group > 0 or d.resid_mod > 0:
         return EPI_GENERIC
-    gl = (_ACT["gelu"], _ACT["quick_gelu"])
+    gl = (_ACT["gelu"], _ACT["quick_gelu"], _ACT["gelu_dbyte"], _ACT["quick_gelu_dbyte"])
     if (d.act and d.act not in gl) or (d.dact and d.dact not in gl) or (d.act and d.dact and d.act != d.dact):
         return EPI_GENERIC
-    quick = _ACT["quick_gelu"] in (d.act, d.dact)
-    m = ((EPI_QUICK if quick else 0) | (EPI_BIAS if d.bias else 0) | (EPI_AUX_OUT if d.aux_out else 0) | (EPI_GELU if d.act else 0) | (EPI_DGELU if d.dact else 0) |
+    quick = _ACT["quick_gelu"] in (d.act, d.dact) or _ACT["quick_gelu_dbyte"] in (d.act, d.dact)
+    dbyte = max(d.act, d.dact) >= _ACT["gelu_dbyte"]
+    m = ((EPI_DBYTE if dbyte else 0) | (EPI_QUICK if quick else 0) | (EPI_BIAS if d.bias else 0) | (EPI_AUX_OUT if d.aux_out else 0) | (EPI_GELU if d.act else 0) | (EPI_DGELU if d.dact else 0) |
          (EPI_RESID if d.resid else 0) | (EPI_RESIDT if (d.residT and not d.resid_lo8) else 0) | (EPI_OUT32 if d.out32 else 0) | (EPI_OUTT if d.outT else 0) |
          (EPI_RESID_LN if ((d.resid or d.resid_lo8) and d.resid_ln_stats) else 0) | (EPI_ROWSUM if d.rowsum_out else 0) | (EPI_LNFOLD if d.lnfold_sums else 0) |
          (EPI_RESID_LO if d.resid_lo8 else 0) | (EPI_OUT_LO if d.out_lo8 else 0))
@@ -337,6 +358,7 @@
     tn, tc = ("bf16", "DF16b") if dtype == torch.bfloat16 else ("float", "f")
     mi = lambda v: f"Li{v}E" if v >= 0 else f"Lin{-v}E"
     if cfg == 12:
+        m = m if m in _PERSIST_SPECIALISED else EPI_GENERIC
         return f"gemm_tn_persist_kernel<{tn},{m}>", f"gemm_tn_persist_kernelI{tc}{mi(m)}E"
     if cfg in (8, 13, 14, 24):
         bm, nbuf = (256, 4) if cfg == 8 else ((256, 5) if cfg == 24 else ((128, 4) if cfg == 13 else (128, 3)))
@@ -503,6 +525,16 @@
     return t[lo:hi] if t.dim() < 3 else t[:, lo:hi]
 
 
+def _check_dact_byte(dt, N, act, dact, aux_in, aux_out):
+    for name, t, code in (("aux_in", aux_in, dact), ("aux_out", aux_out, act)):
+        byte_code, byte_plane = code in _DBYTE.values(), t is not None and t.dtype == torch.uint8
+        if byte_code != byte_plane or (byte_code and dt != torch.bfloat16):
+            raise UiaError(f"gemm {name}: a uint8 derivative-byte plane and the codes {sorted(_DBYTE.values())} go together, on bf16 operands "
+                           f"(got {name} {None if t is None else t.dtype}, activation {code!r}, operands {dt})")
+        if byte_plane and (N % 8 or t.dim() != 2 or t.stride(0) % 8 or t.data_ptr() % 8):
+            raise UiaError(f"gemm {name}: a derivative-byte plane needs N % 8 == 0 and 8-byte aligned rows (N = {N}, stride {t.stride()}, address % 8 = {t.data_ptr() % 8})")
+
+
 def gemm(a, w, *, bias=None, act=None, dact=None, aux_in=None, aux_out=None, resid=None, resid_mod=0, resid_row_off=0,
          resid_t=None, out_group=0, out_t=None, out32=None, alpha=1.0, tile_cfg=0, resid_ln=None, rowsum=None, lnfold=None, drop=None, a2=None,
          resid3=None, out_lo=None):
@@ -517,6 +549,7 @@
             raise UiaError(f"gemm: a2 operand {tuple(t2.shape)} does not match [groups, {M}, {w.K2}] with {w.N} columns in groups of {gcols}")
     else:
         M, (N, K) = (a.rows if is_kb(a) else a.shape[0]), (w.row if isinstance(w, PackedW) else w).shape
+    _check_dact_byte(a.dtype, N, act, dact, aux_in, aux_out)
     plan = plan_gemm(M, N, K, a.element_size(), num_cus(a.device.index) if a.is_cuda else 0, tile_cfg,
                      **_plan_facts(a, w, act, dact, aux_out, out_group, resid_mod, drop, alpha, out_t, out32, resid, resid_t, rowsum, lnfold, resid_ln))
     if len(plan) == 1:
@@ -609,7 +642,9 @@
     if bias is not None:
         assert bias.dtype == torch.float32 and bias.numel() == d.N
         d.bias = _p(bias)
-    for name, t, want in (("aux_in", aux_in, a.dtype), ("aux_out", aux_out, a.dtype), ("resid_t", resid_t, a.dtype),
+    if launch is None:
+        _check_dact_byte(a.dtype, d.N, act, dact, aux_in, aux_out)
+    for name, t, want in (("aux_in", aux_in, torch.uint8 if dact in _DBYTE.values() else a.dtype), ("aux_out", aux_out, torch.uint8 if act in _DBYTE.values() else a.dtype), ("resid_t", resid_t, a.dtype),
                           ("resid", resid, torch.float32), ("out32", out32, torch.float32)):
         if t is not None and t.dtype != want:
             raise UiaError(f"gemm {name} must be {want}, got {t.dtype}")
@@ -672,7 +707,7 @@
         e0.record()
         check(lib().uia_gemm(_stream(), _code(a.dtype), C.byref(d), tile_cfg), "uia_gemm")
         e1.record()
-        nbytes = esz * (d.M * d.K + d.N * d.K) + d.M * d.N * (esz * sum(t is not None for t in (aux_in, aux_out, resid_t, out_t))
+        nbytes = esz * (d.M * d.K + d.N * d.K) + d.M * d.N * (esz * sum(t is not None for t in (resid_t, out_t)) + sum(t.element_size() for t in (aux_in, aux_out) if t is not None)
                                                              + 4 * sum(t is not None for t in (resid, out32)) + 3 * (resid3 is not None) + 1 * (out_lo is not None))
         mask = epi_mask_of(d)
         if not (tile_cfg & 255) and base_cfg != 23:
```

Result: no change. 6856 (median of 4 runs) (+0.1%).
